# edin-dal/sdqlpy

Hardware: AMD Instinct MI355X
Metric: tpch_q1_q3_q5_sf10_rows_per_sec (higher is better)
Workload: dtype f64; 1 GPU; TPCH Q1+Q3+Q5 SF=10 per GPU (BASELINE metric: Q1/Q3/Q5 at SF=10; q1 = configs[1], q3 = configs[2]); partitioning=none

## Files before the change

sdqlpy_amd/csrc/sdqh_hip.hip:

```cpp
#include <hip/hip_runtime.h>

#include <algorithm>
#include <atomic>
#include <chrono>
#include <cmath>
#include <cstdio>
#include <cstdlib>
#include <cstring>
#include <string>
#include <thread>
#include <type_traits>
#include <map>
#include <vector>

#include "sdqh_host.hpp"

using namespace sdqh_host;

static int ensure_index(sdqh_ctx* ctx, sdqh_table* tb);

namespace sdqh_host {

int fail(sdqh_ctx* ctx, int code, const std::string& msg) {
    if (ctx) ctx->err = msg;
    return code;
}

void* pool_alloc(sdqh_ctx* ctx, size_t bytes) {
    bytes = std::max<size_t>(256, (bytes + 255) & ~(size_t)255);
    int best = -1;
    for (size_t i = 0; i < ctx->pool.size(); ++i) {
        PoolBlock& b = ctx->pool[i];
        if (b.free && b.size >= bytes && b.size <= bytes * 2 + (1u << 20) && (best < 0 || b.size < ctx->pool[(size_t)best].size)) best = (int)i;
    }
    if (best >= 0) { PoolBlock& b = ctx->pool[(size_t)best]; b.free = false; b.alloc_seq = ctx->launch_seq; b.fill_use = false; b.graph_owner = ctx->capturing ? ctx->capture_tag : nullptr; return b.ptr; }
    void* p = nullptr;
    if (hipMalloc(&p, bytes) != hipSuccess) {
        for (auto& b : ctx->pool) if (b.free && b.ptr) { (void)hipFree(b.ptr); b.ptr = nullptr; }
        ctx->pool.erase(std::remove_if(ctx->pool.begin(), ctx->pool.end(), [](const PoolBlock& b) { return b.ptr == nullptr; }), ctx->pool.end());
        if (hipMalloc(&p, bytes) != hipSuccess) { (void)hipGetLastError(); return nullptr; }
    }
    { PoolBlock nb{p, bytes, false}; nb.alloc_seq = ctx->launch_seq; nb.graph_owner = ctx->capturing ? ctx->capture_tag : nullptr; ctx->pool.push_back(nb); }
    return p;
}
void pool_free(sdqh_ctx* ctx, void* p) {
    if (!p) return;
    for (auto& b : ctx->pool) if (b.ptr == p) { if (b.graph_owner) return; b.free = true; for (int h = 0; h < b.nhabits; ++h) b.habits[h].clean = false; if (!b.fill_use) b.nhabits = 0; return; }
}

void* attach_alloc(sdqh_ctx* ctx, const sdqh_column* c, size_t bytes) {
    sdqh_ctx* h = c->home ? c->home : ctx;
    if (h != ctx && h->stream) (void)hipStreamSynchronize(h->stream);
    return pool_alloc(h, bytes);
}
void attach_free(sdqh_ctx* ctx, const sdqh_column* c, void* p) { pool_free(c->home ? c->home : ctx, p); }

hipEvent_t next_event(sdqh_ctx* ctx) {
    if (ctx->event_next == ctx->event_pool.size()) { hipEvent_t e; (void)hipEventCreate(&e); ctx->event_pool.push_back(e); }
    return ctx->event_pool[ctx->event_next++];
}
void call_begin(sdqh_ctx* ctx) {
    if (ctx->nested) return;
    if (ctx->profiling != 2) { ctx->prof.clear(); ctx->event_next = 0; }
    ctx->call_timed = false;
    if (ctx->profiling != 1) return;
    (void)hipEventRecord(ctx->call_begin, ctx->stream);
}
void call_end(sdqh_ctx* ctx) {
    if (ctx->nested || ctx->profiling != 1) return;
    (void)hipEventRecord(ctx->call_end, ctx->stream);
    ctx->call_timed = true;
}

int sync_stream(sdqh_ctx* ctx) {
    if (ctx->capturing) return fail(ctx, SDQH_ERR_UNSUPPORTED, "a call that waits for the device cannot be recorded into a plan graph");
    bool done = false;
    if (ctx->opt_spin_sync && !ctx->compile_only) {
        if (!ctx->sync_flag) {
            void* p = nullptr;
            if (hipHostMalloc(&p, 64, hipHostMallocDefault) == hipSuccess) { ctx->sync_flag = static_cast<volatile uint32_t*>(p); *ctx->sync_flag = 0; }
            else { (void)hipGetLastError(); ctx->opt_spin_sync = 0; }
        }
        if (ctx->sync_flag) {
            const uint32_t seq = ++ctx->sync_seq;
            if (hipStreamWriteValue32(ctx->stream, const_cast<uint32_t*>(ctx->sync_flag), seq, 0) == hipSuccess) {
// ... 515 lines not shown
    if (!ctx || !ms) return SDQH_ERR_INVALID;
    if (!ctx->call_timed) { *ms = 0.0; return SDQH_OK; }
    HIP_TRY(ctx, hipEventSynchronize(ctx->call_end));
    float f = 0;
    HIP_TRY(ctx, hipEventElapsedTime(&f, ctx->call_begin, ctx->call_end));
    *ms = f;
    return SDQH_OK;
}
int sdqh_set_profiling(sdqh_ctx* ctx, int mode) {
    if (!ctx || mode < 0 || mode > 2) return SDQH_ERR_INVALID;
    ctx->profiling = mode; ctx->prof.clear(); ctx->event_next = 0;
    return SDQH_OK;
}
int sdqh_set_profile_filter(sdqh_ctx* ctx, const char* kernel_name) {
    if (!ctx) return SDQH_ERR_INVALID;
    ctx->prof_filter = kernel_name ? kernel_name : "";
    return SDQH_OK;
}
int sdqh_profile_count(const sdqh_ctx* ctx) { return ctx ? (int)ctx->prof.size() : 0; }
int sdqh_profile_entry(const sdqh_ctx* cctx, int i, const char** name, double* ms) {
    sdqh_ctx* ctx = const_cast<sdqh_ctx*>(cctx);
    if (!ctx || i < 0 || i >= (int)ctx->prof.size() || !name || !ms) return SDQH_ERR_INVALID;
    ProfEntry& e = ctx->prof[(size_t)i];
    if (e.ms == 0.0) { (void)hipEventSynchronize(e.e1); float f = 0; if (hipEventElapsedTime(&f, e.e0, e.e1) == hipSuccess) e.ms = f; }
    *name = e.name; *ms = e.ms;
    return SDQH_OK;
}
int sdqh_profile_entry_bytes(const sdqh_ctx* ctx, int i, int64_t* model_bytes) {
    if (!ctx || i < 0 || i >= (int)ctx->prof.size() || !model_bytes) return SDQH_ERR_INVALID;
    *model_bytes = ctx->prof[(size_t)i].model_bytes;
    return SDQH_OK;
}
void* sdqh_stream(const sdqh_ctx* ctx) { if (ctx) const_cast<sdqh_ctx*>(ctx)->stream_exported = true; return ctx ? (void*)ctx->stream : nullptr; }
int sdqh_set_option(sdqh_ctx* ctx, const char* name, int64_t value) {
    if (!ctx || !name) return SDQH_ERR_INVALID;
    const std::string n(name);
    if (n == "resident_cap" && value >= 1 && value <= 8) ctx->opt_resident_cap = (int)value;
    else if (n == "async_copies" && (value == 0 || value == 1)) ctx->opt_async_copies = (int)value;
    else if (n == "resident_stream" && value >= 1 && value <= 8) ctx->opt_resident_stream = (int)value;
    else if (n == "probe_chunk" && value >= 1 && value <= 64) ctx->opt_probe_chunk = (int)value;
    else if (n == "probe_unroll" && (value == 1 || value == 2 || value == 4)) ctx->opt_probe_unroll = (int)value;
    else if (n == "stage_batch" && (value == 2 || value == 4 || value == 8)) ctx->opt_stage_batch = (int)value;
    else if (n == "stage_eager" && (value == 0 || value == 1)) ctx->opt_stage_eager = (int)value;
    else if (n == "stage_eager_pay" && (value == 0 || value == 1)) ctx->opt_stage_eager_pay = (int)value;
    else if (n == "stage_waves_per_cu" && value >= 4 && value <= 64) ctx->opt_stage_waves_per_cu = (int)value;
    else if (n == "direct_index" && (value == 0 || value == 1)) ctx->opt_direct_index = (int)value;
    else if (n == "row_pack" && (value == 0 || value == 1)) ctx->opt_row_pack = (int)value;
    else if (n == "cluster_pack" && value >= 0 && value <= 2) ctx->opt_cluster_pack = (int)value;
    else if (n == "cluster_list" && (value == 0 || value == 1)) ctx->opt_cluster_list = (int)value;
    else if (n == "x_driven" && value >= 0 && value <= (1 << 20)) ctx->opt_x_driven = (int)value;
    else if (n == "delta8" && (value == 0 || value == 1)) ctx->opt_delta8 = (int)value;
    else if (n == "word_pairs" && (value == 0 || value == 1)) ctx->opt_word_pairs = (int)value;
    else if (n == "coarse_kb" && value >= 0 && value <= 96) ctx->opt_coarse_kb = (int)value;
    else if (n == "lookup_pipeline" && value >= -1 && value <= 1) ctx->opt_lookup_pipeline = (int)value;
    else if (n == "probe_pipeline" && value >= 0 && value <= 1) ctx->opt_probe_pipeline = (int)value;
    else if (n == "lookup_debug") ctx->opt_lookup_debug = (int)value;
    else if (n == "fuse_small" && value >= 0 && value <= 1) ctx->opt_fuse_small = (int)value;
    else if (n == "lds_key_set" && value >= 0 && value <= 1) ctx->opt_lds_key_set = (int)value;
    else if (n == "fill_ahead" && value >= 0 && value <= 1) { ctx->opt_fill_ahead = (int)value; for (auto& b : ctx->pool) b.nhabits = 0; }
    else if (n == "str_rows" && (value == 0 || value == 32 || value == 64)) ctx->opt_str_rows = (int)value;
    else if (n == "rank_increasing" && value >= 0 && value <= 1) ctx->opt_rank_increasing = (int)value;
    else if (n == "feature_min_rows" && value >= 0) ctx->opt_feature_min_rows = value;
    else if (n == "narrow" && value >= 0 && value <= 1) ctx->opt_narrow = (int)value;
    else if (n == "tight" && value >= 0 && value <= 1) ctx->opt_tight = (int)value;
    else if (n == "spin_sync" && value >= 0 && value <= 1) ctx->opt_spin_sync = (int)value;
    else if (n == "vstage" && value >= 0 && value <= 1) ctx->opt_vstage = (int)value;
    else if (n == "side_streams" && value >= 0 && value <= 1) ctx->opt_side_streams = (int)value;
    else if (n == "side_priority" && value >= 0 && value <= 1) ctx->opt_side_priority = (int)value;
    else if (n == "copy_kernel" && value >= 0 && value <= 4096) ctx->opt_copy_kernel = (int)value;
    else if (n == "copy_nt" && value >= 0 && value <= 1) ctx->opt_copy_nt = (int)value;
    else if (n == "x_waves" && value >= 0 && value <= 256) ctx->opt_x_waves = (int)value;
    else if (n == "window" && value >= 0 && value <= 1) ctx->opt_window = (int)value;
    else if (n == "lane_int" && value >= 0 && value <= 1) ctx->opt_lane_int = (int)value;
    else if (n == "row_index" && value >= 0 && value <= 1) ctx->opt_row_index = (int)value;
    else if (n == "lane_resident" && value >= 1 && value <= 4) ctx->opt_lane_resident = (int)value;
    else if (n == "async_result" && value >= 0 && value <= 1) ctx->opt_async_result = (int)value;
    else if (n == "stage_pipeline" && value >= 0 && value <= 1) ctx->opt_stage_pipeline = (int)value;
    else if (n == "span_index" && value >= 0 && value <= 1) ctx->opt_span_index = (int)value;
    else if (n == "dense_increasing" && value >= 0 && value <= 1) ctx->opt_dense_increasing = (int)value;
    else if (n == "packed_slots" && (value == 0 || value == 1)) ctx->opt_packed_slots = (int)value;
    else if (n == "grouped_index" && (value == 0 || value == 1)) ctx->opt_grouped_index = (int)value;
    else if (n == "grouped_pairs" && (value == 0 || value == 1)) ctx->opt_grouped_pairs = (int)value;
    else if (n == "index_inline" && (value == 0 || value == 1)) ctx->opt_index_inline = (int)value;
    else if (n == "groupby_regs" && (value == 0 || value == 4 || value == 8)) ctx->opt_groupby_regs = (int)value;
    else if (n == "hash_filter" && (value == 0 || value == 1)) ctx->opt_hash_filter = (int)value;
    else if (n == "pack_ordered" && (value == 0 || value == 1)) ctx->opt_pack_ordered = (int)value;
    else if (n == "pool_trim" && value == 1) {
        if (ctx->compile_only) return SDQH_OK;
        if (ctx->capturing) return fail(ctx, SDQH_ERR_UNSUPPORTED, "set_option: pool_trim inside a recording");
        (void)hipSetDevice(ctx->device);
        if (hipStreamSynchronize(ctx->stream) != hipSuccess) { (void)hipGetLastError(); return fail(ctx, SDQH_ERR_DEVICE, "pool_trim: the stream failed"); }
        for (auto& b : ctx->pool) if (b.free && b.ptr && !b.graph_owner) { (void)hipFree(b.ptr); b.ptr = nullptr; }
        ctx->pool.erase(std::remove_if(ctx->pool.begin(), ctx->pool.end(), [](const PoolBlock& b) { return b.ptr == nullptr; }), ctx->pool.end());
    }
    else return fail(ctx, SDQH_ERR_INVALID, "set_option: unknown option or value out of range: " + n);
    return SDQH_OK;
}

int sdqh_memory_stats(sdqh_ctx* ctx, int64_t* out, int n) {
    if (!ctx || !out || n < 4) return fail(ctx, SDQH_ERR_INVALID, "memory_stats: bad arguments");
    int64_t used = 0, cached = 0, graphs = 0, blocks = 0;
    for (const auto& b : ctx->pool) {
        if (!b.ptr) continue;
        ++blocks;
        if (b.graph_owner) graphs += (int64_t)b.size;
        if (b.free && !b.graph_owner) cached += (int64_t)b.size; else used += (int64_t)b.size;
    }
    out[0] = used; out[1] = cached; out[2] = graphs; out[3] = blocks;
    return SDQH_OK;
}

static int new_column(sdqh_ctx* ctx, int64_t nrows, int dtype, int width, sdqh_column** out) {
    if (!ctx || !out || nrows < 0) return fail(ctx, SDQH_ERR_INVALID, "column: bad arguments");
    if (dtype != SDQH_I64 && dtype != SDQH_F64 && dtype != SDQH_STR) return fail(ctx, SDQH_ERR_INVALID, "column: bad dtype");
    if (dtype == SDQH_STR && width < 1) return fail(ctx, SDQH_ERR_INVALID, "column: STR needs width >= 1");
    sdqh_column* c = new sdqh_column();
    c->home = ctx;
    c->nrows = nrows; c->dtype = dtype; c->width = dtype == SDQH_STR ? width : 0;
    *out = c;
    return SDQH_OK;
}

int sdqh_column_alloc(sdqh_ctx* ctx, int64_t nrows, int dtype, int width, sdqh_column** out) {
    if (int rc = new_column(ctx, nrows, dtype, width, out)) return rc;
    sdqh_column* c = *out;
    (void)hipSetDevice(ctx->device);
    c->data = pool_alloc(ctx, (size_t)nrows * c->row_bytes() + 64);
    c->owned = true;
    if (!c->data) { delete c; *out = nullptr; return fail(ctx, SDQH_ERR_NOMEM, "column_alloc: out of device memory"); }
    return SDQH_OK;
}

static void staging_copy(void* dst, const void* src, size_t n) {
    const unsigned hw = std::thread::hardware_concurrency();
    const size_t parts = n < ((size_t)4 << 20) ? 1 : std::min<size_t>(8, std::max<unsigned>(1, hw / 2));
    if (parts <= 1) { std::memcpy(dst, src, n); return; }
    std::vector<std::thread> th;
    const size_t per = ((n / parts) + 4095) & ~(size_t)4095;
    for (size_t k = 1; k < parts; ++k) {
        const size_t b = std::min(n, k * per), e = std::min(n, (k + 1) * per);
        if (e > b) th.emplace_back([=] { std::memcpy(static_cast<char*>(dst) + b, static_cast<const char*>(src) + b, e - b); });
    }
    std::memcpy(dst, src, std::min(n, per));
    for (auto& t : th) t.join();
}

int sdqh_column_upload(sdqh_ctx* ctx, const void* host, int64_t nrows, int dtype, int width, sdqh_column** out) {
    if (nrows > 0 && !host) return fail(ctx, SDQH_ERR_INVALID, "column_upload: null host pointer");
    if (int rc = sdqh_column_alloc(ctx, nrows, dtype, width, out)) return rc;
    sdqh_column* c = *out;
    const size_t bytes = (size_t)nrows * c->row_bytes();
    size_t off = 0; int i = 0;
    while (off < bytes) {
        const size_t n = std::min(STAGING_BYTES, bytes - off);
        if (ctx->staging_busy[i]) { HIP_TRY(ctx, hipEventSynchronize(ctx->staging_done[i])); ctx->staging_busy[i] = false; }
        staging_copy(ctx->staging[i], static_cast<const char*>(host) + off, n);
        HIP_TRY(ctx, hipMemcpyAsync(static_cast<char*>(c->data) + off, ctx->staging[i], n, hipMemcpyHostToDevice, ctx->stream));
        HIP_TRY(ctx, hipEventRecord(ctx->staging_done[i], ctx->stream));
        ctx->staging_busy[i] = true;
        off += n; i ^= 1;
    }
    for (int k = 0; k < 2; ++k) if (ctx->staging_busy[k]) { HIP_TRY(ctx, hipEventSynchronize(ctx->staging_done[k])); ctx->staging_busy[k] = false; }
    return SDQH_OK;
}

int sdqh_column_wrap(sdqh_ctx* ctx, void* device_ptr, int64_t nrows, int dtype, int width, sdqh_column** out) {
// ... 252 lines not shown
        const int g = order[i];
        if (out_keys) for (int k = 0; k < nkeys; ++k) out_keys[i * nkeys + k] = (int64_t)((hk[g] >> (32 * k)) & 0xFFFFFFFFull);
        if (out_values) for (int k = 0; k < SDQH_TUPLE_MAX_VALUES; ++k) out_values[i * SDQH_TUPLE_MAX_VALUES + k] = k < nv ? ha[g * 4 + k] : 0.0;
        if (out_counts) out_counts[i] = hc[g];
    }
    *out_ngroups = ng;
    return SDQH_OK;
}

static void table_release(sdqh_ctx* ctx, sdqh_table* t) {
    for (void* p : t->owned) pool_free(ctx, p);
    t->owned.clear();
}
static void* table_alloc(sdqh_ctx* ctx, sdqh_table* t, size_t bytes) {
    void* p = pool_alloc(ctx, bytes);
    if (p) t->owned.push_back(p);
    return p;
}

static int setup_stage(sdqh_ctx* ctx, sdqh_table* tb, int64_t nrows, const sdqh_column* key, int npay, const sdqh_column* const* payload, int batch, int waves_per_cu = 24) {
    DevStage& st = tb->stage;
    std::memset(&st, 0, sizeof(st));
    const int64_t target_segs = (int64_t)ctx->num_cu * waves_per_cu;
    int64_t seg_rows = (nrows + target_segs - 1) / target_segs;
    const int64_t gran = (int64_t)WAVE * ROWS_PER_LOAD * std::max(1, batch);
    seg_rows = std::max<int64_t>(gran, (seg_rows + gran - 1) / gran * gran);
    if (seg_rows >= ((int64_t)1 << 31)) return fail(ctx, SDQH_ERR_UNSUPPORTED, "build: more than 2^31 rows per staging segment");
    st.seg_rows = seg_rows;
    st.nseg = (int32_t)std::max<int64_t>(1, (nrows + seg_rows - 1) / seg_rows);
    st.npay = npay;
    const size_t col_bytes = (size_t)std::max<int64_t>(nrows, 1) * 8 + 64;
    st.key = static_cast<int64_t*>(table_alloc(ctx, tb, col_bytes));
    st.src_key = static_cast<const int64_t*>(key->data);
    bool ok = st.key != nullptr;
    for (int p = 0; p < npay && ok; ++p) {
        st.pay[p] = static_cast<int64_t*>(table_alloc(ctx, tb, col_bytes));
        st.src_pay[p] = static_cast<const int64_t*>(payload[p]->data);
        ok = st.pay[p] != nullptr;
    }
    st.seg_count = static_cast<uint32_t*>(table_alloc(ctx, tb, (size_t)st.nseg * 4 + 64));
    st.shits = static_cast<uint32_t*>(table_alloc(ctx, tb, (size_t)std::max<int64_t>(nrows, 1) * 4 + 64));
    ok = ok && st.seg_count != nullptr && st.shits != nullptr;
    st.acc_stride = 4;
    if (ok && tb->accumulate) { st.sacc = static_cast<double*>(table_alloc(ctx, tb, (size_t)std::max<int64_t>(nrows, 1) * 32 + 64)); ok = st.sacc != nullptr; }
    if (!ok) return fail(ctx, SDQH_ERR_NOMEM, "out of device memory for the build stage");
    return SDQH_OK;
}

static void prefill_refs(sdqh_ctx* ctx, sdqh_table* tb, FillList* fl) {
    if (!tb->bm || tb->dev.bm_shift != 0) return;
    const size_t rows = (size_t)std::max<int64_t>(tb->nrows_build, 1);
    if (rows * 4 > ((size_t)8 << 20)) return;
    uint32_t* dense = static_cast<uint32_t*>(table_alloc(ctx, tb, rows * 4 + 64));
    if (!dense) return;
    tb->dev.dense_ref = dense; tb->refs_prefilled = true;
    fl->add(dense, (rows * 4 + 15) & ~(size_t)15, 0xFF);
    const size_t range = (size_t)tb->nwords * 32;
    if (ctx->opt_span_index && tb->dev.lin_rb == 0 && range * 4 <= ((size_t)2 << 20)) {
        uint32_t* span = static_cast<uint32_t*>(table_alloc(ctx, tb, range * 4 + 64));
        if (span) { tb->span = span; fl->add(span, range * 4, 0xFF); }
    }
}

static int ensure_index(sdqh_ctx* ctx, sdqh_table* tb) {
    if (tb->index_built || tb->bitmap_only) return SDQH_OK;
    if (tb->dev.grp_first) { tb->index_built = true; return SDQH_OK; }
    const unsigned seg_grid = (unsigned)((tb->stage.nseg + TPB / WAVE - 1) / (TPB / WAVE));
    const size_t rows = (size_t)std::max<int64_t>(tb->nrows_build, 1);
    if (tb->bm && tb->dev.bm_shift == 0 && tb->stage.wrow) {
        LAUNCH(ctx, "k_wrow_fixup", k_wrow_fixup, (unsigned)((tb->stage.nseg + TPB - 1) / TPB), tb->stage, tb->wexc, tb->hdr);
        tb->dev.wprefix = tb->stage.wrow; tb->dev.dense_ref = nullptr; tb->dev.wexc = tb->wexc;
        hipError_t er = hipGetLastError();
        if (er != hipSuccess) return fail(ctx, SDQH_ERR_DEVICE, std::string("table index launch: ") + hipGetErrorString(er));
        tb->index_built = true;
        return SDQH_OK;
    }
    if (tb->bm && tb->dev.bm_shift == 0) {
        const int nblocks = (int)((tb->nwords + RANK_BLOCK_WORDS - 1) / RANK_BLOCK_WORDS);
        uint32_t* wprefix = static_cast<uint32_t*>(table_alloc(ctx, tb, tb->nwords * 4 + 64));
        uint32_t* dense = tb->refs_prefilled ? tb->dev.dense_ref : static_cast<uint32_t*>(table_alloc(ctx, tb, rows * 4 + 64));
        if (!wprefix || !dense) return fail(ctx, SDQH_ERR_NOMEM, "table index: out of device memory");
        tb->dev.wprefix = wprefix; tb->dev.dense_ref = dense;
        if (nblocks == 1 && seg_grid == 1 && tb->refs_prefilled && ctx->opt_fuse_small) {
            LAUNCH(ctx, "k_index_small", k_index_small, 1u, tb->bm, tb->nwords, wprefix, tb->stage, tb->dev, tb->span);
            if (tb->span) tb->dev.dense_arr = tb->span;
            hipError_t es = hipGetLastError();
            if (es != hipSuccess) return fail(ctx, SDQH_ERR_DEVICE, std::string("table index launch: ") + hipGetErrorString(es));
            tb->index_built = true;
            return SDQH_OK;
        }
        if (nblocks == 1 && ctx->opt_fuse_small && (tb->refs_prefilled || tb->keys_unique) && tb->nwords <= (uint64_t)RANK_BLOCK_WORDS) {
            LAUNCH(ctx, "k_index_medium", k_index_medium, seg_grid, tb->bm, (uint32_t)tb->nwords, wprefix, tb->stage, tb->dev, tb->span);
            if (tb->span) tb->dev.dense_arr = tb->span;
            hipError_t em = hipGetLastError();
            if (em != hipSuccess) return fail(ctx, SDQH_ERR_DEVICE, std::string("table index launch: ") + hipGetErrorString(em));
            tb->index_built = true;
            return SDQH_OK;
        }
        LAUNCH(ctx, "k_rank_words", k_rank_words, (unsigned)nblocks, tb->bm, tb->nwords, wprefix, tb->stage.seg_count, tb->stage.nseg, tb->hdr);
        if (!tb->refs_prefilled && !tb->keys_unique) LAUNCH(ctx, "k_fill_refs", k_fill_refs, (unsigned)ctx->num_cu * 2, tb->stage, tb->dev);
        LAUNCH(ctx, "k_insert_direct", k_insert_direct, seg_grid, tb->stage, tb->dev, tb->span);
        if (tb->span) tb->dev.dense_arr = tb->span;
    } else {
        const bool packed = ctx->opt_packed_slots && tb->npay >= 1 && tb->capmax <= (1ull << 27);
        int64_t* keys = nullptr; uint32_t* rowref = nullptr; int64_t* slots = nullptr;
        if (packed) slots = static_cast<int64_t*>(table_alloc(ctx, tb, (tb->capmax + 2) * 32));
        else { keys = static_cast<int64_t*>(table_alloc(ctx, tb, (tb->capmax + 2) * 8)); rowref = static_cast<uint32_t*>(table_alloc(ctx, tb, (tb->capmax + 2) * 4)); }
        if (packed ? !slots : (!keys || !rowref)) return fail(ctx, SDQH_ERR_NOMEM, "table index: out of device memory");
        tb->dev.keys = keys; tb->dev.rowref = rowref; tb->dev.slots = slots;
        uint32_t* hf = nullptr;
        if (ctx->opt_hash_filter) {
            const uint64_t bits = std::max<uint64_t>(std::min<uint64_t>(tb->capmax, HF_MAX_CAP) << HF_SHIFT, 1024);
            hf = static_cast<uint32_t*>(table_alloc(ctx, tb, (size_t)(bits / 8) + 64));
            if (!hf) (void)hipGetLastError();
        }
        tb->dev.hf = hf;
        LAUNCH(ctx, "k_clear", k_clear, (unsigned)ctx->num_cu * 4, tb->stage.seg_count, tb->stage.nseg, tb->capmax, tb->hdr, keys, rowref, slots, hf);
        LAUNCH(ctx, "k_insert", k_insert, seg_grid, tb->stage, tb->dev);
        LAUNCH(ctx, "k_insert_fixup", k_insert_fixup, seg_grid, tb->stage, tb->dev);
        if (packed) LAUNCH(ctx, "k_insert_repack", k_insert_repack, seg_grid, tb->stage, tb->dev);
    }
    hipError_t e = hipGetLastError();
    if (e != hipSuccess) return fail(ctx, SDQH_ERR_DEVICE, std::string("table index launch: ") + hipGetErrorString(e));
    tb->index_built = true;
    return SDQH_OK;
}

static int build_dense(sdqh_ctx* ctx, int64_t nrows, const sdqh_column* key, int npayload, const sdqh_column* const* payload,
                       int64_t lo, int64_t hi, int accumulate, sdqh_table** out) {
    sdqh_table* tb = new sdqh_table();
    tb->npay = npayload; tb->nrows_build = nrows; tb->index_built = true; tb->accumulate = accumulate != 0;
    DevStage& st = tb->stage;
    std::memset(&st, 0, sizeof(st));
    const int64_t target_segs = (int64_t)ctx->num_cu * ctx->opt_stage_waves_per_cu;
    const int64_t gran = (int64_t)WAVE * ROWS_PER_LOAD * 8;
    int64_t seg_rows = (nrows + target_segs - 1) / target_segs;
    st.seg_rows = std::max<int64_t>(gran, (seg_rows + gran - 1) / gran * gran);
    st.nseg = (int32_t)std::max<int64_t>(1, (nrows + st.seg_rows - 1) / st.seg_rows);
    st.npay = npayload;
    st.key = const_cast<int64_t*>(static_cast<const int64_t*>(key->data));
    for (int p = 0; p < npayload; ++p) st.pay[p] = const_cast<int64_t*>(static_cast<const int64_t*>(payload[p]->data));
    const uint64_t range = (uint64_t)(hi - lo) + 1;
    st.seg_count = static_cast<uint32_t*>(table_alloc(ctx, tb, (size_t)st.nseg * 4 + 64));
    st.shits = static_cast<uint32_t*>(table_alloc(ctx, tb, (size_t)nrows * 4 + 64));
    tb->hdr = static_cast<TableHeader*>(table_alloc(ctx, tb, sizeof(TableHeader)));
    const size_t acc_bytes = accumulate ? (size_t)nrows * 32 : 0;
    if (accumulate) {
        st.acc_stride = 4;
        st.sacc = static_cast<double*>(table_alloc(ctx, tb, acc_bytes + 64));
        if (!st.sacc) { table_release(ctx, tb); delete tb; return fail(ctx, SDQH_ERR_NOMEM, "dense build: out of device memory"); }
        tb->dev.sacc = st.sacc; tb->dev.acc_stride = 4;
    }
    const bool increasing = ctx->opt_dense_increasing && column_is_increasing(ctx, const_cast<sdqh_column*>(key));
    const int64_t* kc = static_cast<const int64_t*>(key->data);
    const unsigned grid = (unsigned)std::min<int64_t>((nrows + TPB - 1) / TPB, (int64_t)ctx->num_cu * 8);
    if (increasing && ctx->opt_rank_increasing && (range * 4 > ((uint64_t)16 << 20) || ctx->opt_feature_min_rows == 0)) {
        tb->nwords = (range + 31) / 32;
        tb->bm = static_cast<uint32_t*>(table_alloc(ctx, tb, tb->nwords * 4 + 64));
        uint32_t* wprefix = static_cast<uint32_t*>(table_alloc(ctx, tb, tb->nwords * 4 + 64));
        uint32_t* wpair = ctx->opt_word_pairs ? static_cast<uint32_t*>(table_alloc(ctx, tb, tb->nwords * 8 + 64)) : nullptr;
        if (!st.seg_count || !st.shits || !tb->hdr || !tb->bm || !wprefix) { table_release(ctx, tb); delete tb; return fail(ctx, SDQH_ERR_NOMEM, "dense build: out of device memory"); }
        st.hdr = tb->hdr;
        tb->dev.hdr = tb->hdr; tb->dev.shits = st.shits; tb->dev.bm_lo = lo; tb->dev.bm_hi = hi; tb->dev.bm = tb->bm; tb->dev.bm_shift = 0; tb->dev.wprefix = wprefix;
        tb->dev.wpair = reinterpret_cast<const unsigned long long*>(wpair);
        for (int p = 0; p < npayload; ++p) tb->dev.pay[p] = st.pay[p];
        call_begin(ctx);
        { FillList fl; fl.add(tb->hdr, sizeof(TableHeader), 0); fl.add(st.shits, (size_t)nrows * 4, 0); fl.add(tb->bm, tb->nwords * 4, 0); if (wpair) fl.add(wpair, tb->nwords * 8, 0); if (accumulate) fl.add(st.sacc, acc_bytes, 0); launch_fill(ctx, fl); }
// ... 752 lines not shown
int sdqh_build(sdqh_ctx* ctx, int64_t nrows, const sdqh_filter* filter, int nlookups, const sdqh_lookup* lookups,
               int nkey, const sdqh_source* key, int npayload, const sdqh_source* payload, int accumulate, sdqh_table** out) {
    if (!ctx || nrows < 0 || !out || nkey < 1 || nkey > 2 || !key || npayload < 0 || npayload > SDQH_MAX_PAYLOAD || (npayload && !payload))
        return fail(ctx, SDQH_ERR_INVALID, "build: bad arguments");
    if (nrows >= 0xFFFFFFFEll) return fail(ctx, SDQH_ERR_UNSUPPORTED, "build: build side limited to 2^32-2 rows per GPU");
    (void)hipSetDevice(ctx->device);
    DevFilter f; DevLookups L; DevBuildSpec spec;
    std::memset(&spec, 0, sizeof(spec));
    bool composite = nkey == 2;
    if (int rc = make_filter(ctx, nrows, filter, nullptr, &f)) return rc;
    call_begin(ctx);
    if (int rc = make_lookups(ctx, nrows, nlookups, lookups, &L, &composite)) return rc;
    spec.nkey = nkey; spec.npay = npayload;
    for (int k = 0; k < nkey; ++k) if (int rc = make_source(ctx, key[k], nrows, nlookups, lookups, nlookups, "build key", &spec.key[k])) return rc;
    for (int p = 0; p < npayload; ++p) if (int rc = make_source(ctx, payload[p], nrows, nlookups, lookups, nlookups, "build payload", &spec.pay[p])) return rc;
    int64_t lo = 0, hi = -1; bool want_bm = false;
    if (nrows > 0 && key[0].kind == SDQH_SRC_COLUMN && key[0].col->dtype == SDQH_I64) {
        if (int rc = ensure_minmax(ctx, const_cast<sdqh_column*>(key[0].col))) return rc;
        lo = key[0].col->mn; hi = key[0].col->mx;
        if (hi >= lo && lo > INT64_MIN / 2 && hi < INT64_MAX / 2) {
            const uint64_t range = (uint64_t)(hi - lo) + 1;
            want_bm = range <= (1ull << 31) && range <= 64ull * (uint64_t)std::max<int64_t>(nrows, 1024);
            if (nkey == 2 && (lo < 0 || hi > 0xFFFFFFFFll)) want_bm = false;
        }
    }
    int64_t lin_rb = 0, lin_b0 = 0; uint64_t lin_bits = 0;
    if (want_bm && nkey == 2 && ctx->opt_direct_index && key[1].kind == SDQH_SRC_COLUMN && key[1].col->dtype == SDQH_I64) {
        if (int rc = ensure_minmax(ctx, const_cast<sdqh_column*>(key[1].col))) return rc;
        const int64_t blo = key[1].col->mn, bhi = key[1].col->mx;
        if (bhi >= blo && blo >= 0 && bhi <= 0xFFFFFFFFll) {
            const uint64_t ra = (uint64_t)(hi - lo) + 1, rb = (uint64_t)(bhi - blo) + 1;
            if (rb <= (1ull << 31) / ra && ra * rb <= 64ull * (uint64_t)std::max<int64_t>(nrows, 1024)) { lin_rb = (int64_t)rb; lin_b0 = blo; lin_bits = ra * rb; }
        }
    }
    const bool grouped = ctx->opt_grouped_index && ctx->opt_direct_index && want_bm && nkey == 2 && !lin_rb && nrows > 1 && nrows < ((int64_t)1 << 31) &&
                         hi < ((int64_t)1 << 31) && !key[0].col->transient && column_is_nondecreasing(ctx, const_cast<sdqh_column*>(key[0].col));
    sdqh_table* tb = new sdqh_table();
    tb->npay = npayload; tb->accumulate = accumulate != 0; tb->nrows_build = nrows;
    if (nkey == 1 && nrows > 0 && key[0].kind == SDQH_SRC_COLUMN && key[0].col->dtype == SDQH_I64 && column_is_increasing(ctx, const_cast<sdqh_column*>(key[0].col))) tb->keys_unique = true;
    if (nkey == 2 && nrows > 0 && key[0].kind == SDQH_SRC_COLUMN && key[1].kind == SDQH_SRC_COLUMN && key[0].col->nrows == nrows && key[1].col->nrows == nrows &&
        columns_pair_increasing(ctx, const_cast<sdqh_column*>(key[0].col), const_cast<sdqh_column*>(key[1].col))) tb->pack_unique = true;
    sdqh_column fake; fake.data = nullptr;
    const sdqh_column* fakes[SDQH_MAX_PAYLOAD] = {&fake, &fake, &fake, &fake};
    int rc = setup_stage(ctx, tb, nrows, &fake, npayload, fakes, nrows >= (int64_t)ctx->num_cu * 24 * 512 ? BUILD_LB : 1);
    uint64_t capmax = 1024;
    while (capmax < 2 * (uint64_t)std::max<int64_t>(nrows, 1)) capmax <<= 1;
    tb->capmax = capmax;
    int* flags = nullptr;
    if (!rc) {
        tb->hdr = static_cast<TableHeader*>(table_alloc(ctx, tb, sizeof(TableHeader)));
        flags = static_cast<int*>(table_alloc(ctx, tb, 64));
        if (want_bm && ctx->opt_direct_index) { tb->nwords = lin_rb ? (lin_bits + 31) / 32 : ((uint64_t)(hi - lo) + 32) / 32; tb->bm = static_cast<uint32_t*>(table_alloc(ctx, tb, tb->nwords * 4 + 64)); }
        if (!tb->hdr || !flags || (tb->nwords && !tb->bm)) rc = fail(ctx, SDQH_ERR_NOMEM, "build: out of device memory");
    }
    uint32_t* grp_first = nullptr;
    const size_t grp_cells = grouped ? (size_t)(hi - lo) + 1 : 0;
    if (!rc && grouped && tb->bm) grp_first = static_cast<uint32_t*>(table_alloc(ctx, tb, grp_cells * 4 + 64));
    if (!rc) {
        tb->dev.hdr = tb->hdr; tb->dev.shits = tb->stage.shits; tb->dev.sacc = tb->stage.sacc; tb->dev.acc_stride = tb->stage.acc_stride;
        if (grp_first) {
            tb->stage.grp_first = grp_first;
            tb->dev.grp_first = grp_first; tb->dev.grp_key = tb->stage.key; tb->dev.grp_kstride = 1; tb->dev.grp_seg_rows = tb->stage.seg_rows;
            if (npayload >= 1 && ctx->opt_grouped_pairs) {
                int64_t* kp = static_cast<int64_t*>(table_alloc(ctx, tb, ((size_t)nrows + 8) * 16 + 64));
                if (kp) { tb->stage.grp_kp = kp; tb->dev.grp_key = kp; tb->dev.grp_kstride = 2; }
            } tb->dev.grp_cap = nrows + 1;
        }
        const int shift = (nkey == 2 && !(tb->bm && lin_rb)) ? 32 : 0;
        tb->dev.bm = tb->bm; tb->dev.bm_lo = lo; tb->dev.bm_hi = hi; tb->dev.bitmap_only = 0; tb->dev.bm_shift = shift;
        for (int p = 0; p < npayload; ++p) tb->dev.pay[p] = tb->stage.pay[p];
        tb->stage.bm = tb->bm; tb->stage.bm_lo = lo; tb->stage.bm_hi = hi; tb->stage.hdr = tb->hdr; tb->stage.bm_shift = shift;
        if (tb->bm && lin_rb) { tb->dev.lin_rb = tb->stage.lin_rb = lin_rb; tb->dev.lin_b0 = tb->stage.lin_b0 = lin_b0; }
        const unsigned seg_grid = (unsigned)((tb->stage.nseg + TPB / WAVE - 1) / (TPB / WAVE));
        FillList fl; fl.add(tb->hdr, sizeof(TableHeader), 0); fl.add(flags, 8, 0); if (tb->bm) fl.add(tb->bm, tb->nwords * 4, 0); prefill_refs(ctx, tb, &fl);
        if (grp_first) fl.add(grp_first, grp_cells * 4, 0xFF);
        DevFill pre; std::memset(&pre, 0, sizeof(pre));
        prune_clean(ctx, &fl);
        if (seg_grid == 1 && ctx->opt_fuse_small && fl.most <= ((uint64_t)1 << 20) && fl.f.n <= FILL_MAX) pre = fl.pre(); else launch_fill(ctx, fl);
        DevIndexInline ix; std::memset(&ix, 0, sizeof(ix));
        if (seg_grid == 1 && ctx->opt_fuse_small && ctx->opt_index_inline && tb->bm && shift == 0 && tb->refs_prefilled && (tb->nwords + RANK_BLOCK_WORDS - 1) / RANK_BLOCK_WORDS == 1) {
            uint32_t* wprefix = static_cast<uint32_t*>(table_alloc(ctx, tb, tb->nwords * 4 + 64));
            if (wprefix) {
                tb->dev.wprefix = wprefix;
                ix.t = tb->dev; ix.wprefix = wprefix; ix.span = tb->span; ix.nwords = tb->nwords; ix.on = 1;
            }
        }
        hipError_t e;
        with_scan_filter(f, [&](auto FC) {
            using FCT = decltype(FC);
            if constexpr (std::is_same_v<FCT, FCfg<1, 0, 0, 0>> || std::is_same_v<FCT, FCfg<0, 0, 0, 0>>) {
                const bool eager0 = nlookups > 0 && lookups[0].key[0].kind == SDQH_SRC_COLUMN && lookups[0].key[0].col->dtype == SDQH_I64;
                if (ctx->opt_narrow && nrows >= ctx->opt_feature_min_rows && (eager0 || f.ni == 1)) {
                    const int32_t* nkey0 = eager0 ? static_cast<const int32_t*>(ensure_narrow(ctx, const_cast<sdqh_column*>(lookups[0].key[0].col))) : nullptr;
                    const int32_t* npred0 = f.ni == 1 ? static_cast<const int32_t*>(ensure_narrow(ctx, const_cast<sdqh_column*>(filter->ipred[0].col))) : nullptr;
                    if ((!eager0 || nkey0) && (f.ni != 1 || npred0)) {
                        auto kern = k_build_lookup<FCT, true>;
                        LAUNCH(ctx, "k_build_lookup", kern, seg_grid, f, L, spec, tb->stage, nrows, flags, nkey0, npred0, pre, ix);
                        return SDQH_OK;
                    }
                }
            }
            auto kern = k_build_lookup<FCT>;
            LAUNCH(ctx, "k_build_lookup", kern, seg_grid, f, L, spec, tb->stage, nrows, flags, static_cast<const int32_t*>(nullptr), static_cast<const int32_t*>(nullptr), pre, ix);
            return SDQH_OK;
        });
        if (ix.on) { if (tb->span) tb->dev.dense_arr = tb->span; tb->index_built = true; }
        call_end(ctx);
        e = hipGetLastError();
        if (e != hipSuccess) rc = fail(ctx, SDQH_ERR_DEVICE, std::string("build launch: ") + hipGetErrorString(e));
        auto packs = [&](const sdqh_source& src) {
            if (src.kind != SDQH_SRC_COLUMN || !src.col || src.col->dtype != SDQH_I64) return false;
            sdqh_column* c = const_cast<sdqh_column*>(src.col);
            return ensure_minmax(ctx, c) == SDQH_OK && c->nrows > 0 && c->mn >= 0 && c->mx <= 0xFFFFFFFFll;
        };
        bool proven = composite;
        if (composite && !rc) {
            if (nkey == 2) proven = proven && packs(key[0]) && packs(key[1]);
            for (int l = 0; l < nlookups && proven; ++l) if (lookups[l].nkey == 2) proven = packs(lookups[l].key[0]) && packs(lookups[l].key[1]);
        }
        if (!rc && composite && !proven) {
            e = hipMemcpyAsync(ctx->result_host, flags, 4, hipMemcpyDeviceToHost, ctx->stream);
            if (e != hipSuccess) rc = fail(ctx, SDQH_ERR_DEVICE, hipGetErrorString(e));
            if (!rc) rc = sync_stream(ctx);
            if (!rc && (*static_cast<const int*>(ctx->result_host) & 2)) rc = fail(ctx, SDQH_ERR_UNSUPPORTED, "build: composite key part outside [0, 2^32)");
        }
    }
    if (rc) { table_release(ctx, tb); delete tb; return rc; }
    *out = tb;
    return SDQH_OK;
}

static int lookup_aggregate_launch(sdqh_ctx* ctx, int64_t nrows, const sdqh_filter* filter, int nlookups, const sdqh_lookup* lookups,
                                   int nkeys, const sdqh_source* keys, int tuple_shape, const sdqh_source* operands, void* block, bool device_block) {
    (void)hipSetDevice(ctx->device);
    const int nops = tuple_nops(tuple_shape), nv = tuple_nv(tuple_shape);
    if (nops < 0) return fail(ctx, SDQH_ERR_UNSUPPORTED, "unknown tuple shape");
    DevFilter f; DevLookups L; DevAggSpec spec;
    std::memset(&spec, 0, sizeof(spec));
    bool composite = false;
    if (int rc = make_filter(ctx, nrows, filter, nullptr, &f)) return rc;
    call_begin(ctx);
    if (int rc = make_lookups(ctx, nrows, nlookups, lookups, &L, &composite)) return rc;
    spec.nkeys = nkeys; spec.shape = tuple_shape;
    for (int k = 0; k < nkeys; ++k) if (int rc = make_source(ctx, keys[k], nrows, nlookups, lookups, nlookups, "group key", &spec.key[k])) return rc;
    for (int j = 0; j < nops; ++j) if (int rc = make_source(ctx, operands[j], nrows, nlookups, lookups, nlookups, "tuple operand", &spec.op[j])) return rc;
    L.debug = ctx->opt_lookup_debug;
    L.pipeline = 0;
    if (nlookups > 0 && lookups[0].key[0].kind == SDQH_SRC_COLUMN && lookups[0].key[0].col->dtype == SDQH_I64)
        L.pipeline = ctx->opt_lookup_pipeline >= 0 ? ctx->opt_lookup_pipeline : (column_is_clustered(ctx, const_cast<sdqh_column*>(lookups[0].key[0].col)) ? 1 : 0);
    const int32_t* cluster_key32 = nullptr;
    size_t coarse_lds = 0;
    if (ctx->opt_row_pack && nlookups > 0 && nrows > 0 && nrows >= ctx->opt_feature_min_rows) {
        std::vector<DevSource*> srcs;
        for (int l = 0; l < nlookups; ++l) for (int k = 0; k < L.l[l].nkey; ++k) srcs.push_back(&L.l[l].key[k]);
        for (int k = 0; k < nkeys; ++k) srcs.push_back(&spec.key[k]);
        for (int j = 0; j < nops; ++j) srcs.push_back(&spec.op[j]);
        std::vector<const void*> cols;
        for (DevSource* sr : srcs) if (sr->kind == SDQH_SRC_COLUMN && std::find(cols.begin(), cols.end(), (const void*)sr->col) == cols.end()) cols.push_back(sr->col);
        if (cols.size() >= 5 && cols.size() <= (size_t)MAX_PACK && (size_t)nrows * cols.size() * 8 <= ((size_t)48 << 30)) {
            const int k = (int)((cols.size() + 1) & ~(size_t)1);
            const void* order_col = nullptr;
            sdqh_column* kc0 = (lookups[0].key[0].kind == SDQH_SRC_COLUMN && lookups[0].key[0].col->dtype == SDQH_I64) ? const_cast<sdqh_column*>(lookups[0].key[0].col) : nullptr;
            const sdqh_table* t0 = lookups[0].table;
            const bool unfiltered = f.nc == 0 && f.ns == 0 && f.nf == 0 && f.ni == 0;
            const bool part_bm = t0->bm && !t0->dev.lin_rb && (lookups[0].nkey == 1 ? t0->dev.bm_shift == 0 : t0->dev.bm_shift != 0);
            if (ctx->opt_cluster_pack && ctx->opt_narrow && kc0 && unfiltered && part_bm && !kc0->transient && nrows < ((int64_t)1 << 32) &&
                (nrows >= 4 * ctx->opt_feature_min_rows || ctx->opt_feature_min_rows == 0) && (ctx->opt_cluster_pack == 2 || !column_is_clustered(ctx, kc0)) && ensure_minmax(ctx, kc0) == SDQH_OK)
                order_col = kc0->data;
            sdqh_ctx::RowPack* found = nullptr;
// ... 523 lines not shown
```

sdqlpy_amd/csrc/sdqh_host.hpp:

```cpp
#pragma once
#include <hip/hip_runtime.h>

#include <atomic>
#include <map>
#include <string>
#include <vector>

#include "sdqh.h"
#include "sdqh_kernels.hpp"

namespace sdqh_host {

struct FillHabit { size_t off, bytes; int byte; bool clean; };
struct PoolBlock {
    void* ptr; size_t size; bool free;
    FillHabit habits[4] = {};
    int nhabits = 0;
    uint64_t alloc_seq = 0;
    bool fill_use = false;
    const void* graph_owner = nullptr;
};
struct ProfEntry { const char* name; hipEvent_t e0, e1; double ms; int64_t model_bytes; };

constexpr size_t STAGING_BYTES = 32u << 20;
constexpr size_t RESULT_BYTES = 64u << 10;

}

using namespace sdqh;

struct sdqh_ctx {
    int device = 0;
    sdqh_ctx* parent = nullptr;
    std::vector<sdqh_ctx*> children;
    const void* capture_tag = nullptr;
    struct HostInit { void* p; uint64_t value; int bytes; };
    std::vector<HostInit> capture_inits;
    bool capturing = false;
    bool dying = false;
    bool compile_only = false;
    int num_cu = 256;
    hipStream_t stream = nullptr;
    bool stream_exported = false;
    std::string err;
    std::vector<sdqh_host::PoolBlock> pool;
    void* staging[2] = {nullptr, nullptr};
    hipEvent_t staging_done[2] = {nullptr, nullptr};
    bool staging_busy[2] = {false, false};
    void* result_host = nullptr;
    void* result_dev = nullptr;
    void* bulk_host = nullptr;
    size_t bulk_bytes = 0;
    std::map<const char*, size_t> host_blocks;
    void* count_host = nullptr;
    hipEvent_t call_begin = nullptr, call_end = nullptr;
    bool call_timed = false;
    int profiling = 0;
    std::string prof_filter;
    std::vector<sdqh_host::ProfEntry> prof;
    int64_t next_model_bytes = 0;
    std::vector<hipEvent_t> event_pool;
    size_t event_next = 0;
    const void* lds_hint[SDQH_MAX_GROUPKEYS] = {nullptr, nullptr};
    int threads = 1;
    std::vector<std::pair<const void*, int>> occupancy;
    int opt_resident_cap = 6;
    int opt_async_copies = 0;
    int opt_probe_chunk = 1;
    int opt_resident_stream = 2;
    int opt_probe_unroll = PROBE_UNROLL;
    int opt_stage_batch = STAGE_BATCH;
    int opt_stage_eager = 1;
    int nested = 0;
    int opt_stage_eager_pay = 0;
    int opt_stage_waves_per_cu = 12;
    int opt_direct_index = 1;
    int opt_packed_slots = 1;
    int opt_lookup_pipeline = -1;
    int opt_lookup_debug = 0;
    size_t rd_clean_ff = 0; int64_t rd_clean_zero_off = -1;
    int opt_fill_ahead = 1;
    uint64_t launch_seq = 0;
    int opt_lds_key_set = 1;
    int opt_fuse_small = 1;
    int opt_str_rows = 0;
    int opt_rank_increasing = 1;
    int64_t opt_feature_min_rows = 1 << 20;
    bool in_groupby_key = false;
    int opt_vstage = 1;
    int opt_tight = 1;
    hipStream_t side[2] = {nullptr, nullptr};
    hipEvent_t side_ev[4] = {nullptr, nullptr, nullptr, nullptr};
    int opt_side_streams = 1;
    int opt_side_priority = 1;
    int opt_copy_kernel = 0;
    int opt_copy_nt = 1;
    int opt_row_index = 1;
    int opt_grouped_index = 1;
    int opt_grouped_pairs = 1;
    int opt_index_inline = 1;
    int opt_lane_int = 1;
    int opt_lane_resident = 2;
    int opt_window = 0;
    int opt_x_driven = 64;
    int opt_word_pairs = 0;
    int opt_delta8 = 1;
    int opt_x_waves = 0;
    void* rs_dev[2] = {nullptr, nullptr}; size_t rs_bytes[2] = {0, 0};
    hipEvent_t rs_copied[2] = {nullptr, nullptr}; bool rs_used[2] = {false, false};
    int rs_cur = 0; bool rs_pending = false;
    hipEvent_t rs_ready = nullptr;
    volatile uint32_t* sync_flag = nullptr; uint32_t sync_seq = 0; int opt_spin_sync = 1;
    int opt_async_result = 1;
    int opt_narrow = 1;
    int opt_stage_pipeline = 0;
    int opt_span_index = 1;
    int opt_dense_increasing = 1;
    int opt_probe_pipeline = 0;
    const void* coarse_stat_col = nullptr; uint64_t* coarse_stat = nullptr;
    unsigned long long* coarse_count_dev = nullptr; uint64_t coarse_stat_bits_pending = 0; int coarse_skipped = 0; int64_t coarse_stat_build_rows = -1;
    int opt_coarse_kb = 64;
    int opt_row_pack = 1;
    struct RowPack { std::vector<const void*> cols; int64_t nrows; int k; void* data; const void* order_col = nullptr; void* key32 = nullptr;
                     void* lb = nullptr; int64_t key_lo = 0, key_hi = -1; };
    std::vector<RowPack> packs;
    int opt_pack_ordered = 1;
    int opt_hash_filter = 1;
    int opt_cluster_list = 1;
    int opt_cluster_pack = 1;
    int opt_groupby_regs = 0;
    const void* g4_hint[SDQH_MAX_GROUPKEYS] = {nullptr, nullptr};
};

inline uint64_t sdqh_next_uid() { static std::atomic<uint64_t> next{1}; return next.fetch_add(1, std::memory_order_relaxed); }

struct sdqh_column {
    uint64_t uid = sdqh_next_uid();
    uint64_t pair_uid = 0; int pair_increasing = -1;
    sdqh_ctx* home = nullptr;
    void* data = nullptr;
    int64_t nrows = 0;
    int dtype = SDQH_I64;
    int width = 0;
    bool owned = false;
    long long* d_minmax = nullptr;
    bool minmax_pending = false, have_minmax = false;
    int clustered = -1;
    void* narrow = nullptr;
    int narrow_state = -1;
    int increasing = -1;
    int nondecreasing = -1;
    int span8 = -1;
    int64_t mn = 0, mx = 0;
    void* code = nullptr;
    int code_width = 0;
    int code_state = -1;
    void* dict = nullptr;
    int ndict = 0;
    std::vector<int64_t> dict_host;
    void* delta8 = nullptr;
    int delta8_state = -1;
    void* run_index = nullptr;
    int run_index_state = -1;
    bool transient = false;
    size_t row_bytes() const { return dtype == SDQH_STR ? (size_t)width * 4 : 8; }
};

struct sdqh_table {
    sdqh::DevTable dev{};
    DevStage stage{};
    TableHeader* hdr = nullptr;
    uint32_t* bm = nullptr;
    int npay = 0;
    bool accumulate = false;
    bool bitmap_only = false;
    int64_t nrows_build = 0;
    uint64_t capmax = 0;
    bool index_built = false;
    uint64_t nwords = 0;
    std::vector<void*> owned;
    uint32_t* span = nullptr;
    bool pack_unique = false;
    bool keys_unique = false;
// ... 86 lines not shown
```

sdqlpy_amd/csrc/sdqh_kernels.hpp:

```cpp
#pragma once
#ifndef __HIPCC_RTC__
#include <hip/hip_runtime.h>
#include <stdint.h>
#endif
#include "sdqh.h"

#if defined(__HIPCC_RTC__) || defined(SDQH_DECLS_ONLY)
#define SDQH_KERNEL template <int SDQH_RTC_UNUSED = 0> __global__
#else
#define SDQH_KERNEL __global__
#endif

namespace sdqh {

constexpr int TPB = 256;
constexpr int WAVE = 64;
constexpr int ROWS_PER_LOAD = 2;
#ifndef SDQH_UNROLL
#define SDQH_UNROLL 2
#endif
#ifndef SDQH_NT_LOADS
#define SDQH_NT_LOADS 1
#endif
#ifndef SDQH_TILE_CHUNK
// ... 1206 lines not shown
                const int off = j * (int)BATCH_ROWS + lane * ROWS_PER_LOAD;
                if (p[j][0]) q_off[at] = (uint16_t)off;
                if (p[j][1]) q_off[at + (p[j][0] ? 1 : 0)] = (uint16_t)(off + 1);
                qn += __popcll(b0) + __popcll(b1);
            }
            __builtin_amdgcn_wave_barrier();
            for (int i0 = 0; i0 < qn; i0 += WAVE) {
                const int i = i0 + lane;
                if (i < qn) {
                    const int64_t row = b + q_off[i];
                    int64_t pay[MAX_STAGE_COLS];
                    const int64_t key = st.src_key[row];
#pragma unroll
                    for (int c = 0; c < MAX_STAGE_COLS; ++c) pay[c] = c < cfg_npay<NPAY>(st.npay) ? st.src_pay[c][row] : 0;
                    stage_store<NPAY>(st, out + i, key, pay);
                }
            }
            __builtin_amdgcn_wave_barrier();
            out += qn;
            continue;
        }
        if (!(EAGER_PAY && full_step)) {
#pragma unroll
            for (int j = 0; j < SB; ++j) {
#pragma unroll
                for (int q = 0; q < 2; ++q) {
                    kx[j][q] = p[j][q] ? st.src_key[r[j] + q] : 0;
#pragma unroll
                    for (int c = 0; c < MAX_STAGE_COLS; ++c) px[j][q][c] = (c < cfg_npay<NPAY>(st.npay) && p[j][q]) ? st.src_pay[c][r[j] + q] : 0;
                }
            }
        }
#pragma unroll
        for (int j = 0; j < SB; ++j) {
            const uint64_t b0 = __ballot(p[j][0]), b1 = __ballot(p[j][1]);
            const int64_t pos0 = out + __popcll(b0 & lt) + __popcll(b1 & lt);
            if (p[j][0]) stage_store<NPAY>(st, pos0, kx[j][0], px[j][0]);
            if (p[j][1]) stage_store<NPAY>(st, pos0 + (p[j][0] ? 1 : 0), kx[j][1], px[j][1]);
            out += __popcll(b0) + __popcll(b1);
        }
    }
    if (lane == 0) st.seg_count[seg] = (uint32_t)(out - begin);
}

SDQH_KERNEL __launch_bounds__(TPB) void k_clear(const uint32_t* __restrict__ seg_count, int nseg, uint64_t capmax,
                                               TableHeader* __restrict__ hdr, int64_t* __restrict__ keys, uint32_t* __restrict__ rowref, int64_t* __restrict__ slots,
                                               uint32_t* __restrict__ hf) {
    __shared__ unsigned long long s_part[TPB];
    unsigned long long t = 0;
    for (int i = threadIdx.x; i < nseg; i += TPB) t += seg_count[i];
    s_part[threadIdx.x] = t;
    __syncthreads();
    for (int off = TPB / 2; off > 0; off >>= 1) { if ((int)threadIdx.x < off) s_part[threadIdx.x] += s_part[threadIdx.x + off]; __syncthreads(); }
    const uint64_t staged = s_part[0];
    uint64_t cap = 1024;
    while (cap < 2 * staged) cap <<= 1;
    if (cap > capmax) cap = capmax;
    if (blockIdx.x == 0 && threadIdx.x == 0) {
        hdr->cap_mask = cap - 1; hdr->staged = staged;
        if (slots) { slots[cap * 4] = EMPTY_KEY; slots[cap * 4 + 3] = (int64_t)NO_ROW; }
        else { keys[cap] = EMPTY_KEY; rowref[cap] = NO_ROW; }
    }
    if (hf) {
        using W = uint32_t __attribute__((ext_vector_type(4)));
        const uint32_t hm = hf_mask_of(cap - 1);
        const uint64_t n16 = ((uint64_t)hm + 1) / 128;
        const uint32_t z = hm == HF_DEGENERATE ? 0xFFFFFFFFu : 0u;
        const W zero = {z, z, z, z};
        W* h4 = reinterpret_cast<W*>(hf);
        for (uint64_t i = (uint64_t)blockIdx.x * TPB + threadIdx.x; i < n16; i += (uint64_t)gridDim.x * TPB) h4[i] = zero;
    }
    using V = long long __attribute__((ext_vector_type(2)));
    if (slots) {
        const V a = {(long long)EMPTY_KEY, 0}, b = {0, (long long)NO_ROW};
        V* s2 = reinterpret_cast<V*>(slots);
        for (uint64_t i = (uint64_t)blockIdx.x * TPB + threadIdx.x; i < cap; i += (uint64_t)gridDim.x * TPB) { s2[2 * i] = a; s2[2 * i + 1] = b; }
        return;
    }
    const V empty = {(long long)EMPTY_KEY, (long long)EMPTY_KEY};
    V* k2 = reinterpret_cast<V*>(keys);
    for (uint64_t i = (uint64_t)blockIdx.x * TPB + threadIdx.x; i < cap / 2; i += (uint64_t)gridDim.x * TPB) k2[i] = empty;
}

__device__ __forceinline__ void rank_words_body(const uint32_t* __restrict__ bm, uint64_t nwords, uint32_t* __restrict__ wprefix,
                                                const uint32_t* __restrict__ seg_count, int nseg, TableHeader* __restrict__ hdr) {
    __shared__ uint32_t s_wave[TPB / WAVE];
    __shared__ uint32_t s_base;
    constexpr int ROWS = RANK_BLOCK_WORDS / (TPB * 4);
    const uint64_t q0 = (uint64_t)blockIdx.x * (RANK_BLOCK_WORDS / 4);
    const uint64_t nquads = (nwords + 3) / 4;
    const int w = threadIdx.x / WAVE, lane = lane_id();
    uint4 quad[ROWS];
    uint32_t excl[ROWS];
    uint32_t running = 0;
#pragma unroll
    for (int r = 0; r < ROWS; ++r) {
        const uint64_t qi = q0 + (uint64_t)r * TPB + threadIdx.x;
        uint4 a = make_uint4(0u, 0u, 0u, 0u);
        if (qi < nquads) {
            a = *reinterpret_cast<const uint4*>(bm + qi * 4);
            const uint64_t wi = qi * 4;
            if (wi + 1 >= nwords) a.y = 0u;
            if (wi + 2 >= nwords) a.z = 0u;
            if (wi + 3 >= nwords) a.w = 0u;
        }
        quad[r] = a;
        const uint32_t mine = (uint32_t)(__popc(a.x) + __popc(a.y) + __popc(a.z) + __popc(a.w));
        uint32_t incl = mine;
#pragma unroll
        for (int off = 1; off < WAVE; off <<= 1) { const uint32_t v = __shfl_up(incl, off, WAVE); if (lane >= off) incl += v; }
        __syncthreads();
        if (lane == WAVE - 1) s_wave[w] = incl;
        __syncthreads();
        uint32_t before = 0, total = 0;
#pragma unroll
        for (int i = 0; i < TPB / WAVE; ++i) { if (i < w) before += s_wave[i]; total += s_wave[i]; }
        excl[r] = running + before + incl - mine;
        running += total;
    }
    uint32_t stg = 0;
    for (int i = blockIdx.x * TPB + threadIdx.x; i < nseg; i += gridDim.x * TPB) stg += seg_count[i];
#pragma unroll
    for (int off = WAVE / 2; off > 0; off >>= 1) stg += __shfl_down(stg, off, WAVE);
    if (lane == 0 && stg) atomicAdd(reinterpret_cast<unsigned long long*>(&hdr->staged), (unsigned long long)stg);
    if (threadIdx.x == 0) s_base = running ? (uint32_t)atomicAdd(reinterpret_cast<unsigned long long*>(&hdr->distinct), (unsigned long long)running) : 0u;
    __syncthreads();
    const uint32_t base = s_base;
#pragma unroll
    for (int r = 0; r < ROWS; ++r) {
        const uint64_t qi = q0 + (uint64_t)r * TPB + threadIdx.x;
        if (qi >= nquads) continue;
        uint4 p;
        p.x = base + excl[r];
        p.y = p.x + (uint32_t)__popc(quad[r].x);
        p.z = p.y + (uint32_t)__popc(quad[r].y);
        p.w = p.z + (uint32_t)__popc(quad[r].z);
        *reinterpret_cast<uint4*>(wprefix + qi * 4) = p;
    }
}
SDQH_KERNEL __launch_bounds__(TPB) void k_rank_words(const uint32_t* __restrict__ bm, uint64_t nwords, uint32_t* __restrict__ wprefix,
                                                    const uint32_t* __restrict__ seg_count, int nseg, TableHeader* __restrict__ hdr) {
    rank_words_body(bm, nwords, wprefix, seg_count, nseg, hdr);
}
SDQH_KERNEL __launch_bounds__(TPB) void k_wrow_fixup(DevStage st, WordExc* __restrict__ exc, TableHeader* __restrict__ hdr) {
    const int s = (int)(blockIdx.x * TPB + threadIdx.x);
    if (s == 0) hdr->has_dups = 0;
    if (s >= st.nseg) return;
    const uint32_t cnt = st.seg_count[s];
    if (!cnt) return;
    const SegFirst f = st.seg_first[s];
    const uint64_t off0 = (uint64_t)(f.key - st.bm_lo);
    const uint32_t w0 = (uint32_t)(off0 >> 5), word = st.bm[w0];
    const uint32_t n_below = __popc(word & ((1u << (off0 & 31)) - 1u));
    if (n_below == 0) {
        if (cnt >= (uint32_t)__popc(word)) st.wrow[w0] = f.pos;
        return;
    }
    int t = s - 1;
    while (t > 0 && st.seg_count[t] == 0) --t;
    WordExc e;
    e.key0 = f.key; e.pos0 = f.pos; e.n0 = n_below; e._pad = 0;
    e.pos_prev = (uint32_t)((int64_t)t * st.seg_rows + (int64_t)st.seg_count[t] - (int64_t)n_below);
    exc[s] = e;
    st.wrow[w0] = ROW_INDEX_EXC | (uint32_t)s;
}
__device__ __forceinline__ bool direct_has_dups(const TableHeader* hdr) { return hdr->staged != hdr->distinct; }
SDQH_KERNEL __launch_bounds__(TPB) void k_fill_refs(DevStage st, DevTable t) {
    if (!direct_has_dups(t.hdr)) return;
    const uint64_t n = t.hdr->distinct;
    for (uint64_t i = (uint64_t)blockIdx.x * TPB + threadIdx.x; i < n; i += (uint64_t)gridDim.x * TPB) t.dense_ref[i] = NO_ROW;
}
__device__ __forceinline__ void insert_direct_body(const DevStage& st, const DevTable& t, uint32_t* __restrict__ span) {
    const int seg = blockIdx.x * (TPB / WAVE) + threadIdx.x / WAVE;
    const bool dups = direct_has_dups(t.hdr);
    if (blockIdx.x == 0 && threadIdx.x == 0) t.hdr->has_dups = dups ? 1u : 0u;
    if (seg >= st.nseg) return;
    const int64_t base = (int64_t)seg * st.seg_rows;
    const uint32_t count = st.seg_count[seg];
    for (uint32_t i = lane_id(); i < count; i += WAVE) {
        const int64_t idx = base + i;
        const int64_t pos = table_find(t, st.key[idx], 0);
        if (pos < 0) continue;
        if (dups) atomicMin(&t.dense_ref[pos], (uint32_t)idx); else t.dense_ref[pos] = (uint32_t)idx;
        if (span) { uint32_t* cell = span + (st.key[idx] - t.bm_lo); if (dups) atomicMin(cell, (uint32_t)idx); else *cell = (uint32_t)idx; }
    }
}
SDQH_KERNEL __launch_bounds__(TPB) void k_insert_direct(DevStage st, DevTable t, uint32_t* __restrict__ span) { insert_direct_body(st, t, span); }
SDQH_KERNEL __launch_bounds__(TPB) void k_index_small(const uint32_t* __restrict__ bm, uint64_t nwords, uint32_t* __restrict__ wprefix, DevStage st, DevTable t, uint32_t* __restrict__ span) {
    rank_words_body(bm, nwords, wprefix, st.seg_count, st.nseg, t.hdr);
    __threadfence();
    __syncthreads();
    insert_direct_body(st, t, span);
}
SDQH_KERNEL __launch_bounds__(TPB) void k_index_medium(const uint32_t* __restrict__ bm, uint32_t nwords, uint32_t* __restrict__ wprefix, DevStage st, DevTable t, uint32_t* __restrict__ span) {
    __shared__ uint32_t s_word[RANK_BLOCK_WORDS], s_pre[RANK_BLOCK_WORDS];
    __shared__ uint32_t s_wave[TPB / WAVE];
    __shared__ uint32_t s_staged;
    constexpr int PER = RANK_BLOCK_WORDS / TPB;
    const int lane = lane_id(), w = threadIdx.x / WAVE;
    for (int i = threadIdx.x; i < RANK_BLOCK_WORDS; i += TPB) s_word[i] = (uint32_t)i < nwords ? bm[i] : 0u;
    if (threadIdx.x == 0) s_staged = 0u;
    __syncthreads();
    uint32_t mine = 0;
#pragma unroll
    for (int j = 0; j < PER; ++j) mine += (uint32_t)__popc(s_word[threadIdx.x * PER + j]);
    uint32_t incl = mine;
#pragma unroll
    for (int off = 1; off < WAVE; off <<= 1) { const uint32_t v = __shfl_up(incl, off, WAVE); if (lane >= off) incl += v; }
    if (lane == WAVE - 1) s_wave[w] = incl;
    uint32_t stg = 0;
    for (int i = threadIdx.x; i < st.nseg; i += TPB) stg += st.seg_count[i];
#pragma unroll
    for (int off = WAVE / 2; off > 0; off >>= 1) stg += __shfl_down(stg, off, WAVE);
    if (lane == 0 && stg) atomicAdd(&s_staged, stg);
    __syncthreads();
    uint32_t before = 0, total = 0;
#pragma unroll
    for (int i = 0; i < TPB / WAVE; ++i) { if (i < w) before += s_wave[i]; total += s_wave[i]; }
    uint32_t run = before + incl - mine;
#pragma unroll
    for (int j = 0; j < PER; ++j) { s_pre[threadIdx.x * PER + j] = run; run += (uint32_t)__popc(s_word[threadIdx.x * PER + j]); }
    __syncthreads();
    const uint32_t staged = s_staged;
    const bool dups = staged != total;
    if (blockIdx.x == 0) {
        for (uint32_t i = threadIdx.x; i < nwords; i += TPB) wprefix[i] = s_pre[i];
        if (threadIdx.x == 0) { t.hdr->staged = staged; t.hdr->distinct = total; t.hdr->has_dups = dups ? 1u : 0u; }
    }
    const int seg = blockIdx.x * (TPB / WAVE) + w;
    if (seg >= st.nseg) return;
    const int64_t base = (int64_t)seg * st.seg_rows;
    const uint32_t count = st.seg_count[seg];
    for (uint32_t i = lane; i < count; i += WAVE) {
        const int64_t idx = base + i;
        const int64_t key = st.key[idx];
        uint64_t off;
        if (!bm_locate(t, key, off) || (off >> 5) >= (uint64_t)RANK_BLOCK_WORDS) continue;
        const uint32_t word = s_word[off >> 5];
        if (!((word >> (off & 31)) & 1u)) continue;
        const uint32_t pos = s_pre[off >> 5] + (uint32_t)__popc(word & ((1u << (off & 31)) - 1u));
        if (dups) atomicMin(&t.dense_ref[pos], (uint32_t)idx); else t.dense_ref[pos] = (uint32_t)idx;
        if (span) { uint32_t* cell = span + (key - t.bm_lo); if (dups) atomicMin(cell, (uint32_t)idx); else *cell = (uint32_t)idx; }
    }
}

SDQH_KERNEL __launch_bounds__(TPB) void k_full_counts(uint32_t* __restrict__ seg_count, int nseg, int64_t seg_rows, int64_t nrows) {
    const int s = blockIdx.x * TPB + threadIdx.x;
    if (s < nseg) { int64_t b = (int64_t)s * seg_rows, e = b + seg_rows; if (e > nrows) e = nrows; seg_count[s] = (uint32_t)(e - b); }
}
SDQH_KERNEL __launch_bounds__(TPB) void k_dense_fill(const int64_t* __restrict__ key, int64_t nrows, int64_t lo, uint32_t* __restrict__ arr) {
    for (int64_t r = (int64_t)blockIdx.x * TPB + threadIdx.x; r < nrows; r += (int64_t)gridDim.x * TPB) arr[key[r] - lo] = (uint32_t)r;
}
SDQH_KERNEL __launch_bounds__(TPB) void k_check_increasing(const int64_t* __restrict__ key, int64_t nrows, int* __restrict__ flag) {
    bool bad = false;
    for (int64_t r = (int64_t)blockIdx.x * TPB + threadIdx.x; r + 1 < nrows; r += (int64_t)gridDim.x * TPB) bad |= key[r] >= key[r + 1];
    if (__ballot(bad) && lane_id() == 0) atomicOr(flag, 1);
}
SDQH_KERNEL __launch_bounds__(TPB) void k_check_nondecreasing(const int64_t* __restrict__ key, int64_t nrows, int* __restrict__ flag) {
    bool bad = false;
    for (int64_t r = (int64_t)blockIdx.x * TPB + threadIdx.x; r + 1 < nrows; r += (int64_t)gridDim.x * TPB) bad |= key[r] > key[r + 1];
    if (__ballot(bad) && lane_id() == 0) atomicOr(flag, 1);
}
SDQH_KERNEL __launch_bounds__(TPB) void k_check_pair_increasing(const int64_t* __restrict__ a, const int64_t* __restrict__ b, int64_t nrows, int* __restrict__ flag) {
    bool bad = false;
    for (int64_t r = (int64_t)blockIdx.x * TPB + threadIdx.x; r + 1 < nrows; r += (int64_t)gridDim.x * TPB) bad |= !(a[r] < a[r + 1] || (a[r] == a[r + 1] && b[r] < b[r + 1]));
    if (__ballot(bad) && lane_id() == 0) atomicOr(flag, 1);
}
constexpr int PAIR_RUN_MAX = 32;
SDQH_KERNEL __launch_bounds__(TPB) void k_check_pair_distinct(const int64_t* __restrict__ a, const int64_t* __restrict__ b, int64_t nrows, int* __restrict__ flag) {
    int bad = 0;
    for (int64_t r = (int64_t)blockIdx.x * TPB + threadIdx.x; r + 1 < nrows; r += (int64_t)gridDim.x * TPB) {
        const int64_t ar = a[r], br = b[r];
        int64_t j = r + 1;
        for (; j < nrows && j <= r + PAIR_RUN_MAX && a[j] == ar; ++j) bad |= b[j] == br ? 1 : 0;
        if (j < nrows && j > r + PAIR_RUN_MAX && a[j] == ar) bad |= 2;
// ... 656 lines not shown
    return 0;
}
template <bool PACKED = false>
__device__ __forceinline__ int run_lookups(const DevLookups& L, int64_t r, uint32_t (&ent)[SDQH_MAX_LOOKUP], const PackRow& pr, bool skip0 = false) {
#pragma unroll
    for (int l = 0; l < SDQH_MAX_LOOKUP; ++l) {
        if (l < L.n && !(l == 0 && skip0)) {
            const DevLookup& lk = L.l[l];
            const int64_t p0 = source_value<PACKED>(lk.key[0], L, r, ent, pr);
            const int64_t p1 = lk.nkey == 2 ? source_value<PACKED>(lk.key[1], L, r, ent, pr) : 0;
            int64_t key;
            if (pack_parts(lk.nkey, p0, p1, key)) return -1;
            const uint64_t mask = (table_is_direct(lk.table) || lk.table.bitmap_only) ? 0 : lk.table.hdr->cap_mask;
            const int64_t pos = table_find(lk.table, key, mask);
            if (pos < 0) return 0;
            ent[l] = lk.table.bitmap_only ? 0u : (lk.table.slots && !table_is_direct(lk.table) ? (uint32_t)pos : table_ref(lk.table, pos));
        }
    }
    return 1;
}
__device__ __forceinline__ bool coarse_may_hit(const DevLookups& L, const uint32_t* s_coarse, int64_t part0) {
    const DevTable& t = L.l[0].table;
    if (part0 < t.bm_lo || part0 > t.bm_hi) return false;
    const uint64_t j = (uint64_t)(part0 - t.bm_lo) >> L.coarse_shift;
    return (s_coarse[j >> 5] >> (j & 31)) & 1u;
}
SDQH_KERNEL __launch_bounds__(TPB) void k_coarsen(const uint32_t* __restrict__ bm, uint64_t nbits, int shift, uint32_t* __restrict__ coarse, int cwords, unsigned long long* __restrict__ set_bits) {
    unsigned long long mine = 0;
    for (int w = blockIdx.x * TPB + threadIdx.x; w < cwords; w += gridDim.x * TPB) {
        uint32_t out = 0;
        for (int b = 0; b < 32; ++b) {
            const uint64_t f0 = ((uint64_t)w * 32 + (uint64_t)b) << shift, f1 = f0 + (1ull << shift);
            bool any = false;
            for (uint64_t f = f0; f < f1 && f < nbits && !any; ) {
                const uint32_t word = bm[f >> 5];
                const uint32_t lo = (uint32_t)(f & 31), span = (uint32_t)min((uint64_t)(32 - lo), f1 - f);
                const uint32_t mask = (span >= 32 ? 0xFFFFFFFFu : ((1u << span) - 1u)) << lo;
                any = (word & mask) != 0u;
                f += span;
            }
            out |= any ? (1u << b) : 0u;
        }
        coarse[w] = out;
        mine += (unsigned long long)__popc(out);
    }
    mine = (unsigned long long)wave_sum_i64((long long)mine);
    if (set_bits && lane_id() == 0 && mine) atomicAdd(set_bits, mine);
}
__device__ __forceinline__ bool first_lookup_may_hit(const DevLookups& L, int64_t part0) {
    const DevTable& t = L.l[0].table;
    if (!t.bm) return true;
    if (L.l[0].nkey == 2 && t.bm_shift == 0) return true;
    if (part0 < t.bm_lo || part0 > t.bm_hi) return false;
    const uint64_t off = (uint64_t)(part0 - t.bm_lo);
    return (t.bm[off >> 5] >> (off & 31)) & 1u;
}

__device__ __forceinline__ bool first_lookup_none(const DevLookups& L) {
    const DevTable& t = L.l[0].table;
    return !t.bm || (L.l[0].nkey == 2 && t.bm_shift == 0);
}
__device__ __forceinline__ uint32_t first_lookup_word(const DevLookups& L, int64_t part0) {
    const DevTable& t = L.l[0].table;
    const bool in = part0 >= t.bm_lo && part0 <= t.bm_hi;
    const uint64_t off = in ? (uint64_t)(part0 - t.bm_lo) : 0;
    return t.bm[off >> 5];
}
__device__ __forceinline__ bool first_lookup_bit(const DevLookups& L, int64_t part0, uint32_t word) {
    const DevTable& t = L.l[0].table;
    const bool in = part0 >= t.bm_lo && part0 <= t.bm_hi;
    return in && ((word >> ((uint64_t)(part0 - t.bm_lo) & 31)) & 1u);
}

constexpr int BUILD_LB = 4;
constexpr int LOOKUP_PU = 2;
constexpr int LBQ_CAP = 64 + BUILD_LB * 128;

struct DevBuildSpec {
    int32_t nkey, npay;
    DevSource key[2];
    DevSource pay[SDQH_MAX_PAYLOAD];
};

struct DevIndexInline { DevTable t; uint32_t* wprefix; uint32_t* span; uint64_t nwords; int32_t on, _pad; };

template <class FC, bool NW>
__device__ __forceinline__ void build_lookup_segment(const DevFilter& f, const DevLookups& L, const DevBuildSpec& spec, const DevStage& st, int64_t nrows, int* __restrict__ flags,
                                                     const int32_t* __restrict__ nkey0, const int32_t* __restrict__ npred0, int32_t* q_row, const int seg) {
    const int64_t* skey0 = NW ? reinterpret_cast<const int64_t*>(nkey0) : L.l[0].key[0].col;
    const int64_t begin = (int64_t)seg * st.seg_rows;
    int64_t end = begin + st.seg_rows; if (end > nrows) end = nrows;
    const int lane = lane_id();
    const uint64_t lt = lanemask_lt();
    constexpr int64_t BATCH_ROWS = WAVE * ROWS_PER_LOAD;
    const bool eager0 = L.n > 0 && L.l[0].key[0].kind == SDQH_SRC_COLUMN;
    DevProbes none; none.n = 0;
    const uint64_t nomask[SDQH_MAX_PROBE] = {0, 0};
    int64_t out = begin;
    int qn = 0;
    bool bad = false;
    auto drain = [&](int first, int count) {
        bool keep = false; int64_t key = 0; int64_t pay[MAX_STAGE_COLS] = {0, 0, 0, 0, 0};
        if (lane < count) {
            const int64_t r = begin + (int64_t)q_row[first + lane];
            uint32_t ent[SDQH_MAX_LOOKUP] = {0, 0, 0};
            const PackRow nopack{};
            const int h = run_lookups(L, r, ent, nopack);
            if (h < 0) bad = true;
            if (h > 0) {
                const int64_t p0 = source_value(spec.key[0], L, r, ent, nopack);
                const int64_t p1 = spec.nkey == 2 ? source_value(spec.key[1], L, r, ent, nopack) : 0;
                if (pack_parts(spec.nkey, p0, p1, key)) bad = true;
                else {
                    keep = true;
#pragma unroll
                    for (int q = 0; q < SDQH_MAX_PAYLOAD; ++q) if (q < spec.npay) pay[q] = source_value(spec.pay[q], L, r, ent, nopack);
                }
            }
        }
        const uint64_t b = __ballot(keep);
        bool opens_run = true;
        if (st.grp_first) {
            const uint64_t lower = b & lt;
            const int prev = lower ? 63 - __builtin_clzll(lower) : lane;
            const int64_t prev_key = __shfl(key, prev, WAVE);
            opens_run = !lower || ((uint64_t)prev_key >> 32) != ((uint64_t)key >> 32);
        }
        if (keep) stage_store<-1>(st, out + __popcll(b & lt), key, pay, opens_run);
        out += __popcll(b);
    };
    auto enqueue = [&](int64_t r, bool p0, bool p1) {
        const uint64_t b0 = __ballot(p0), b1 = __ballot(p1);
        if (b0 | b1) {
            const int at = qn + __popcll(b0 & lt) + __popcll(b1 & lt);
            const int32_t off = (int32_t)(r - begin);
            if (p0) q_row[at] = off;
            if (p1) q_row[at + (p0 ? 1 : 0)] = off + 1;
            qn += __popcll(b0) + __popcll(b1);
        }
    };
    for (int64_t b = begin;;) {
        const bool last = b >= end;
        if (last) {
        } else if (b + BATCH_ROWS * BUILD_LB <= end) {
            int64_t rr[BUILD_LB];
            bool p[BUILD_LB][2];
            Pair<int64_t> k0[BUILD_LB];
#pragma unroll
            for (int j = 0; j < BUILD_LB; ++j) {
                rr[j] = b + (int64_t)j * BATCH_ROWS + (int64_t)lane * ROWS_PER_LOAD;
                p[j][0] = p[j][1] = true;
                if (eager0) k0[j] = loadc<false, NW>(skey0, rr[j], nrows);
            }
            pass_pairs<BUILD_LB, FC, false, false, false, NW>(f, none, rr, nrows, nomask, p, nullptr, nullptr, nullptr, npred0);
            if (eager0) {
#pragma unroll
                for (int j = 0; j < BUILD_LB; ++j) { p[j][0] = p[j][0] && first_lookup_may_hit(L, k0[j].x); p[j][1] = p[j][1] && first_lookup_may_hit(L, k0[j].y); }
            }
#pragma unroll
            for (int j = 0; j < BUILD_LB; ++j) enqueue(rr[j], p[j][0], p[j][1]);
            b += BATCH_ROWS * BUILD_LB;
        } else {
            const int64_t r = b + (int64_t)lane * ROWS_PER_LOAD;
            bool p1b[1][2];
            if (b + BATCH_ROWS <= end) {
                int64_t r1[1] = {r};
                p1b[0][0] = p1b[0][1] = true;
                Pair<int64_t> k1 = {0, 0};
                if (eager0) k1 = load2<false>(L.l[0].key[0].col, r, nrows);
                pass_pairs<1, FC, false>(f, none, r1, nrows, nomask, p1b);
                if (eager0) { p1b[0][0] = p1b[0][0] && first_lookup_may_hit(L, k1.x); p1b[0][1] = p1b[0][1] && first_lookup_may_hit(L, k1.y); }
            } else {
                p1b[0][0] = r < end; p1b[0][1] = r + 1 < end;
                if (p1b[0][0]) p1b[0][0] = row_passes<FC>(f, none, r, nomask);
                if (p1b[0][1]) p1b[0][1] = row_passes<FC>(f, none, r + 1, nomask);
            }
            enqueue(r, p1b[0][0], p1b[0][1]);
            b += BATCH_ROWS;
        }
        int head = 0;
        while (qn - head >= WAVE || (last && qn > head)) {
            const int n = qn - head >= WAVE ? WAVE : qn - head;
            drain(head, n);
            head += n;
        }
        if (last) break;
        if (head) {
            const int left = qn - head;
            int32_t keepv = 0;
            if (lane < left) keepv = q_row[head + lane];
            if (lane < left) q_row[lane] = keepv;
            qn = left;
        }
    }
    if (lane == 0) {
        st.seg_count[seg] = (uint32_t)(out - begin);
        stage_end_segment(st, seg, begin, out - begin);
        if (st.grp_first && seg == 0) st.hdr->has_dups = 1u;
    }
    if (__ballot(bad) && lane == 0) atomicOr(flags, 2);
}

template <class FC, bool NW = false>
__global__ __launch_bounds__(TPB) void k_build_lookup(DevFilter f, DevLookups L, DevBuildSpec spec, DevStage st, int64_t nrows, int* __restrict__ flags,
                                                      const int32_t* __restrict__ nkey0, const int32_t* __restrict__ npred0, DevFill pre, DevIndexInline ix) {
    if (pre.n) { fill_in_block(pre); __syncthreads(); }
    __shared__ int32_t s_row[TPB / WAVE][LBQ_CAP];
    const int seg = blockIdx.x * (TPB / WAVE) + threadIdx.x / WAVE;
    if (seg < st.nseg) build_lookup_segment<FC, NW>(f, L, spec, st, nrows, flags, nkey0, npred0, s_row[threadIdx.x / WAVE], seg);
    if (ix.on) {
        __threadfence();
        __syncthreads();
        rank_words_body(st.bm, ix.nwords, ix.wprefix, st.seg_count, st.nseg, st.hdr);
        __threadfence();
        __syncthreads();
        insert_direct_body(st, ix.t, ix.span);
    }
}

struct DevPackCols { const int64_t* col[MAX_PACK]; int32_t ncols, k; };
SDQH_KERNEL __launch_bounds__(TPB) void k_interleave(DevPackCols c, int64_t nrows, int64_t* __restrict__ out) {
    for (int64_t r = (int64_t)blockIdx.x * TPB + threadIdx.x; r < nrows; r += (int64_t)gridDim.x * TPB) {
        int64_t v[MAX_PACK];
#pragma unroll
        for (int j = 0; j < MAX_PACK; ++j) v[j] = j < c.ncols ? c.col[j][r] : 0;
#pragma unroll
        for (int j = 0; j < MAX_PACK; ++j) if (j < c.k) out[r * c.k + j] = v[j];
    }
}

constexpr int LG_SLOTS = 2 * SDQH_MAX_LOOKUP_GROUPS;

struct DevAggSpec {
    int32_t nkeys, shape;
    DevSource key[SDQH_MAX_GROUPKEYS];
    DevSource op[4];
};

__device__ __forceinline__ int group_slot(unsigned long long* keys, unsigned long long key, bool global) {
    int h = (int)(mix64(key) & (LG_SLOTS - 1));
#pragma unroll 1
    for (int i = 0; i < LG_SLOTS; ++i) {
        unsigned long long cur = global ? __hip_atomic_load(&keys[h], __ATOMIC_RELAXED, __HIP_MEMORY_SCOPE_AGENT) : keys[h];
        if (cur == EMPTY_GROUP) cur = atomicCAS(&keys[h], (unsigned long long)EMPTY_GROUP, key);
        if (cur == EMPTY_GROUP || cur == key) return h;
        h = (h + 1) & (LG_SLOTS - 1);
    }
    return -1;
}

template <int SHAPE, class FC, int BT = TPB, int PUV = LOOKUP_PU, bool NW = false, bool WALK = false>
__global__ __launch_bounds__(BT) void k_lookup_agg(DevFilter f, DevLookups L, DevAggSpec spec, int64_t nrows,
                                                    unsigned long long* __restrict__ gkeys, double* __restrict__ pacc,
                                                    int64_t* __restrict__ pcnt, int* __restrict__ flags, int chunk, const int32_t* __restrict__ nkey0) {
    const int64_t* skey0 = NW ? reinterpret_cast<const int64_t*>(nkey0) : L.l[0].key[0].col;
    constexpr int NOPS = TupleTraits<SHAPE>::NOPS, NV = TupleTraits<SHAPE>::NV;
    constexpr int PU = PUV, TILE = BT * ROWS_PER_LOAD * PU, SUBR = BT * ROWS_PER_LOAD, QCAP = 64 + PU * 128;
    __shared__ unsigned long long s_keys[LG_SLOTS];
    constexpr int NVS = NV > 0 ? NV : 1;
    __shared__ double s_acc[LG_SLOTS][NVS];
    __shared__ unsigned long long s_cnt[LG_SLOTS];
    __shared__ int32_t s_row[BT / WAVE][QCAP];
    __shared__ int s_map[LG_SLOTS];
    __shared__ int s_flags[1];
    for (int i = threadIdx.x; i < LG_SLOTS; i += BT) { s_keys[i] = EMPTY_GROUP; s_cnt[i] = 0; for (int k = 0; k < NVS; ++k) s_acc[i][k] = 0.0; s_map[i] = -1; }
    for (int i = threadIdx.x; i < LG_SLOTS; i += BT) pcnt[(size_t)i * gridDim.x + blockIdx.x] = 0;
    if (threadIdx.x == 0) s_flags[0] = 0;
    __syncthreads();
    constexpr bool COARSE = BT != TPB;
    extern __shared__ __align__(16) uint32_t s_coarse[];
    if constexpr (COARSE) { for (int i = threadIdx.x; i < L.coarse_words; i += BT) s_coarse[i] = L.coarse[i]; __syncthreads(); }
    int32_t* q_row = s_row[threadIdx.x / WAVE];
    const int lane = lane_id();
    const uint64_t lt = lanemask_lt();
    const bool eager0 = L.n > 0 && L.l[0].key[0].kind == SDQH_SRC_COLUMN;
    DevProbes none; none.n = 0;
    const uint64_t nomask[SDQH_MAX_PROBE] = {0, 0};
    int qn = 0;
    const bool skip0 = eager0 && !first_lookup_none(L) && L.l[0].table.bitmap_only && L.l[0].nkey == 1 && L.l[0].table.bm_shift == 0 && L.l[0].table.lin_rb == 0 && !(L.debug & 2);
    int64_t qbase = 0;
    auto drain = [&](int first, int count) {
        if (lane >= count) return;
        if (L.debug & 1) return;
        const int64_t r = qbase + (int64_t)q_row[first + lane];
        uint32_t ent[SDQH_MAX_LOOKUP] = {0, 0, 0};
        PackRow prow{};
        if (L.pack) pack_load(L, r, prow);
        double x[4] = {0, 0, 0, 0}, o[4] = {0, 0, 0, 0};
        if (L.debug & 8) { if (prow.v0 == -12345 && prow.v5 == -777) atomicOr(&s_flags[0], 2); return; }
        const int h = run_lookups<true>(L, r, ent, prow, skip0);
        if (h < 0) atomicOr(&s_flags[0], 2);
        if (h <= 0) return;
        if (L.debug & 4) { if (ent[0] + ent[1] + ent[2] == 0xFFFFFFF0u) atomicOr(&s_flags[0], 2); return; }
        const int64_t k0 = source_value<true>(spec.key[0], L, r, ent, prow);
        const int64_t k1 = spec.nkeys == 2 ? source_value<true>(spec.key[1], L, r, ent, prow) : 0;
#pragma unroll
        for (int j = 0; j < NOPS; ++j) x[j] = __longlong_as_double(source_value<true>(spec.op[j], L, r, ent, prow));
        if (k0 < 0 || k0 > 0xFFFFFFFEll || k1 < 0 || k1 > 0xFFFFFFFEll) { atomicOr(&s_flags[0], 2); return; }
        if (!operand_ranges<NOPS>(f, x)) return;
// ... 719 lines not shown
```

sdqlpy_amd/csrc/sdqh_x.hip:

```cpp
#define SDQH_DECLS_ONLY 1
#include <hip/hip_runtime.h>
#include <hip/hiprtc.h>

#include <dlfcn.h>
#include <sys/stat.h>
#include <unistd.h>

#include <algorithm>
#include <chrono>
#include <cstdio>
#include <cstdlib>
#include <cstring>
#include <fstream>
#include <mutex>
#include <sstream>
#include <string>
#include <vector>

#include "sdqh_host.hpp"
#include "sdqh_xkernels.hpp"

using namespace sdqh_host;

namespace {
// ... 1083 lines not shown
    out << "    template <int H> __device__ __forceinline__ static bool eval_regs(const XArgs& a, const Pair<int64_t> (&s)[" << nsx << "], int64_t r, XOut<NV>& o) {\n";
    if (direct) out << body(1, 0); else out << "        return false;\n";
    out << "    }\n";
    out << "    __device__ __forceinline__ static bool eval_row(const XArgs& a, int64_t r, const int64_t (&sres)[" << nsopx << "], XOut<NV>& o) {\n";
    if (!direct) out << body(0, first_gate); else out << "        return false;\n";
    out << "    }\n};\n";
    const std::string sn = sink_name(sink);
    out << "extern \"C\" __global__ __launch_bounds__(256) void " << entry_name(sink, direct, q8) << "(XArgs a, " << sn << "<P::NV>::Args s, int64_t nrows, int64_t seg_rows, int nseg) {\n";
    if (direct) out << "    x_direct<P, " << sn << ">(a, s, nrows);\n";
    else out << "    " << (q8 ? "x_queue8" : "x_queue") << "<P, " << sn << ", " << (sink == SINK_STAGE ? "true" : "false") << ">(a, s, nrows, seg_rows, nseg);\n";
    out << "}\n";
    return out.str();
}

struct JitState {
    std::mutex mu;
    bool headers_loaded = false; std::string h_abi, h_kernels, h_xkernels, src_dir, cache_dir, why_unusable;
    std::map<std::string, hipFunction_t> kernels;
    int64_t compiled = 0, from_disk = 0;
};
JitState& jit() { static JitState s; return s; }

std::string slurp(const std::string& path) {
    std::ifstream f(path, std::ios::binary);
    if (!f) return std::string();
    std::stringstream ss; ss << f.rdbuf();
    return ss.str();
}
uint64_t fnv1a(const std::string& s, uint64_t h = 1469598103934665603ull) {
    for (unsigned char c : s) { h ^= c; h *= 1099511628211ull; }
    return h;
}

bool load_headers(JitState& J) {
    if (J.headers_loaded) return J.why_unusable.empty();
    J.headers_loaded = true;
    std::string dir;
    if (const char* env = std::getenv("SDQLPY_AMD_CSRC")) dir = env;
    else {
        Dl_info info;
        if (dladdr(reinterpret_cast<const void*>(&sdqh_jit_stats), &info) && info.dli_fname) { dir = info.dli_fname; const size_t at = dir.rfind('/'); dir = at == std::string::npos ? "." : dir.substr(0, at); }
    }
    J.src_dir = dir;
    J.h_kernels = slurp(dir + "/sdqh_kernels.hpp");
    J.h_xkernels = slurp(dir + "/sdqh_xkernels.hpp");
    J.h_abi = slurp(dir + "/../../include/sdqh.h");
    if (J.h_abi.empty()) J.h_abi = slurp(dir + "/sdqh.h");
    if (J.h_kernels.empty() || J.h_xkernels.empty() || J.h_abi.empty()) {
        J.why_unusable = "run-time specialisation needs sdqh_kernels.hpp, sdqh_xkernels.hpp next to libsdqlhip.so and include/sdqh.h (looked in " + dir + ")";
        return false;
    }
    if (const char* env = std::getenv("SDQLPY_AMD_JIT_CACHE")) J.cache_dir = env;
    else J.cache_dir = dir + "/../jit_cache";
    (void)mkdir(J.cache_dir.c_str(), 0777);
    return true;
}

uint64_t structure_hash(const XInfo& x, Sink sink, bool direct) {
    const sdqh_program* p = x.p;
    uint64_t h = 1469598103934665603ull;
    auto mix = [&](uint64_t v) { h ^= v; h *= 0x9E3779B97F4A7C15ull; h ^= h >> 29; };
    mix((uint64_t)sink * 2 + (direct ? 1 : 0)); mix((uint64_t)x.narrow_mask);
    if (x.tight) {
        mix(0x7167ull); mix((uint64_t)x.gather32); mix((x.pref32 ? 1ull : 0ull) | (x.vstage ? 2ull : 0ull) | (x.pwin ? 4ull : 0ull) | (x.pnear ? 8ull : 0ull) | (x.driven ? 16ull : 0ull) | (x.phash ? 32ull : 0ull) | ((uint64_t)(x.ival + 1) << 8));
        for (int c = 0; c < x.ncols; ++c) mix(((uint64_t)(uint32_t)x.enc[c] << 32) | ((uint32_t)(x.affine[c] ? 1 : 0) << 16) | (uint32_t)(x.dict_slot[c] & 0xFFFF));
        for (int k = 0; k < x.p->nops; ++k) mix((uint64_t)(uint8_t)x.irange[k]);
        for (int k = 0; k < x.p->nops; ++k) mix(((uint64_t)(uint32_t)x.cmp_cc[k] << 32) | ((uint32_t)x.cmp_kind[k] << 8) | (uint32_t)(x.cmp_col[k] & 0xFF));
    } mix((uint64_t)p->nops); mix((uint64_t)(int64_t)p->key); mix((uint64_t)(int64_t)x.probe_op);
    for (int k = 0; k < p->nops; ++k) {
        const sdqh_xop& o = p->ops[k];
        mix(((uint64_t)(uint32_t)o.code << 32) | (uint32_t)o.type); mix(((uint64_t)(uint32_t)o.a << 32) | (uint32_t)o.b); mix(((uint64_t)(uint32_t)o.c << 32) | (uint32_t)o.aux);
        mix(((uint64_t)(uint32_t)x.col_of[k] << 32) | (uint32_t)x.tab_of[k]); mix(((uint64_t)(uint32_t)x.const_of[k] << 32) | (uint32_t)x.str_off[k]);
        if (o.code == SDQH_X_DIVI || o.code == SDQH_X_MODI) mix((uint64_t)o.imm_i);
        if (o.code == SDQH_X_STR || o.code == SDQH_X_STRIDX) { mix((uint64_t)o.slen); for (int i = 0; i < o.slen; ++i) mix(o.str[i]); }
        if (o.code == SDQH_X_STR || o.code == SDQH_X_STRIDX || o.code == SDQH_X_CHAR) mix((uint64_t)(o.col ? o.col->width : 0));
    }
    mix((uint64_t)p->ngates); for (int g = 0; g < p->ngates; ++g) mix((uint64_t)p->gates[g]);
    mix((uint64_t)p->nvals); for (int v = 0; v < p->nvals; ++v) mix((uint64_t)p->vals[v]);
    return h;
}

int specialise(sdqh_ctx* ctx, const std::string& source, const std::string& entry, hipFunction_t* fn);

int kernel_for(sdqh_ctx* ctx, const XInfo& x, Sink sink, bool direct, hipFunction_t* fn) {
    JitState& J = jit();
    static const bool no_layouts = std::getenv("SDQLPY_AMD_X_NOLAYOUT") != nullptr;
    uint64_t lay_hash = 0;
    for (int t = 0; t < x.ntabs; ++t) {
        if (ctx->compile_only) { x.lay[t] = 0u; continue; }
        if (int rc = index_ensure(ctx, x.tabs[t])) return rc;
        x.lay[t] = no_layouts ? 0u : x_layout_of(x.tabs[t]->dev, x.tabs[t]->bitmap_only);
        lay_hash = (lay_hash ^ x.lay[t]) * 0x9E3779B97F4A7C15ull + (uint64_t)t;
    }
    char name[64];
    std::snprintf(name, sizeof(name), "s%016llx@%d", (unsigned long long)(structure_hash(x, sink, direct) ^ lay_hash), ctx->device);
    if (!ctx->compile_only) {
        std::lock_guard<std::mutex> lock(J.mu);
        auto hit = J.kernels.find(name);
        if (hit != J.kernels.end()) { *fn = hit->second; return SDQH_OK; }
    }
    if (int rc = specialise(ctx, generate(x, sink, direct), (x.vstage && sink == SINK_STAGE) ? std::string(VSTAGE_ENTRY) : entry_name(sink, direct, x.tight), fn)) return rc;
    std::lock_guard<std::mutex> lock(J.mu);
    J.kernels[name] = *fn;
    return SDQH_OK;
}

int specialise(sdqh_ctx* ctx, const std::string& source_in, const std::string& entry, hipFunction_t* fn) {
    std::string source = source_in;
    if (const char* defs = std::getenv("SDQLPY_AMD_X_DEFINES")) {
        std::istringstream in(defs); std::string tok, head;
        while (in >> tok) { const size_t eq = tok.find('='); head += "#define " + (eq == std::string::npos ? tok + " 1" : tok.substr(0, eq) + " " + tok.substr(eq + 1)) + "\n"; }
        source = head + source;
    }
    JitState& J = jit();
    std::lock_guard<std::mutex> lock(J.mu);
    if (!load_headers(J)) return fail(ctx, SDQH_ERR_DEVICE, J.why_unusable);
    int rtc_major = 0, rtc_minor = 0;
    (void)hiprtcVersion(&rtc_major, &rtc_minor);
    uint64_t h = fnv1a(source);
    h = fnv1a(J.h_xkernels, h); h = fnv1a(J.h_kernels, h); h = fnv1a(J.h_abi, h);
    h = fnv1a("gfx950 rtc " + std::to_string(rtc_major) + "." + std::to_string(rtc_minor), h);
    char name[64];
    std::snprintf(name, sizeof(name), "%016llx", (unsigned long long)h);
    const std::string key = std::string(name) + "@" + std::to_string(ctx->device);
    auto hit = J.kernels.find(key);
    if (hit != J.kernels.end()) { *fn = hit->second; return SDQH_OK; }
    if (const char* dump = std::getenv("SDQLPY_AMD_JIT_DUMP")) if (dump[0] == '2') std::fprintf(stderr, "---- specialised source (%s) ----\n%s\n", entry.c_str(), source.c_str());
    const std::string path = J.cache_dir + "/" + name + ".hsaco";
    std::string code = slurp(path);
    if (!code.empty()) ++J.from_disk;
    else {
        hiprtcProgram prog;
        const char* hs[3] = {J.h_abi.c_str(), J.h_kernels.c_str(), J.h_xkernels.c_str()};
        const char* hn[3] = {"sdqh.h", "sdqh_kernels.hpp", "sdqh_xkernels.hpp"};
        if (hiprtcCreateProgram(&prog, source.c_str(), "sdqh_specialised.hip", 3, hs, hn) != HIPRTC_SUCCESS)
            return fail(ctx, SDQH_ERR_DEVICE, "hiprtcCreateProgram failed");
        const char* opts[] = {"--offload-arch=gfx950", "-O3", "-std=c++17", "-ffp-contract=off", "-munsafe-fp-atomics"};
        const hiprtcResult r = hiprtcCompileProgram(prog, 5, opts);
        if (r != HIPRTC_SUCCESS) {
            size_t n = 0; (void)hiprtcGetProgramLogSize(prog, &n);
            std::string log(n + 1, '\0');
            if (n) (void)hiprtcGetProgramLog(prog, &log[0]);
            (void)hiprtcDestroyProgram(&prog);
            if (std::getenv("SDQLPY_AMD_JIT_DUMP")) std::fprintf(stderr, "---- specialised source ----\n%s\n", source.c_str());
            return fail(ctx, SDQH_ERR_DEVICE, std::string("hiprtc: ") + hiprtcGetErrorString(r) + "\n" + log.substr(0, 4000));
        }
        size_t n = 0; (void)hiprtcGetCodeSize(prog, &n);
        code.resize(n);
        (void)hiprtcGetCode(prog, &code[0]);
        (void)hiprtcDestroyProgram(&prog);
        ++J.compiled;
        if (const char* rdir = std::getenv("SDQLPY_AMD_JIT_RECIPES")) {
            char rn[32]; std::snprintf(rn, sizeof(rn), "%016llx", (unsigned long long)fnv1a(source));
            (void)mkdir(rdir, 0777);
            std::ofstream rf(std::string(rdir) + "/" + rn + ".hip", std::ios::binary);
            rf << source;
        }
        const std::string tmp = path + ".tmp." + std::to_string((long)getpid());
        { std::ofstream f(tmp, std::ios::binary); f.write(code.data(), (std::streamsize)code.size()); }
        (void)std::rename(tmp.c_str(), path.c_str());
    }
    if (ctx->compile_only) return fail(ctx, SDQH_ERR_DEVICE, "compile-only context: kernel specialised (" + std::to_string(code.size()) + " bytes of gfx950 code), not run");
    hipModule_t mod;
    if (hipModuleLoadData(&mod, code.data()) != hipSuccess) { (void)hipGetLastError(); return fail(ctx, SDQH_ERR_DEVICE, "hipModuleLoadData failed for a specialised kernel"); }
    hipFunction_t f;
    if (hipModuleGetFunction(&f, mod, entry.c_str()) != hipSuccess) { (void)hipGetLastError(); return fail(ctx, SDQH_ERR_DEVICE, "specialised kernel has no entry point"); }
    J.kernels[key] = f;
    *fn = f;
    return SDQH_OK;
}

template <class SA> struct Packed { XArgs a; SA s; int64_t nrows; int64_t seg_rows; int32_t nseg; };

int fill_xargs(sdqh_ctx* ctx, const XInfo& x, XArgs* a, int32_t* flags, int64_t key_lo, int64_t key_hi) {
    std::memset(a, 0, sizeof(*a));
    for (int c = 0; c < x.ncols; ++c) { a->col[c] = x.cols[c]->data; a->width[c] = x.cols[c]->width; a->ncol[c] = (((x.narrow_mask | x.gather32) >> c) & 1u) ? x.cols[c]->narrow : nullptr; }
    for (int t = 0; t < x.ntabs; ++t) {
        if (int rc = index_ensure(ctx, x.tabs[t])) return rc;
        a->tab[t] = x.tabs[t]->dev;
    }
    if (x.tight) for (int c = 0; c < x.ncols; ++c) a->dlo[c] = x.dlo[c];
    if (x.tight) for (int c = 0; c < x.ncols; ++c) if (x.enc[c] == ENC_D8) a->dcol[c] = x.cols[c]->delta8;
    if (x.tight) for (int c = 0; c < x.ncols; ++c) if (x.enc[c] >= ENC_C16) { a->code[c] = x.cols[c]->code; a->dict[c] = static_cast<const int64_t*>(x.cols[c]->dict); a->ndict[c] = x.cols[c]->ndict; }
    std::memcpy(a->cc, x.cc, sizeof(x.cc[0]) * (size_t)x.ncc);
    std::memcpy(a->ci, x.ci, sizeof(x.ci[0]) * (size_t)x.nci);
    std::memcpy(a->cf, x.cf, sizeof(x.cf[0]) * (size_t)x.ncf);
    std::memcpy(a->spool, x.spool, sizeof(uint32_t) * (size_t)x.nstr);
    a->flags = flags; a->key_lo = key_lo; a->key_hi = key_hi;
    if (x.driven && x.driven_col >= 0 && x.cols[x.driven_col]->run_index_state == 1) {
        const sdqh_column* kc = x.cols[x.driven_col];
        a->run_index = static_cast<const uint32_t*>(kc->run_index); a->run_lo = kc->mn; a->run_hi = kc->mx; a->driven_ratio = ctx->opt_x_driven;
    }
    return SDQH_OK;
}

struct Geometry { unsigned grid; int64_t seg_rows; int nseg; };
Geometry geometry_tight(sdqh_ctx* ctx, int64_t nrows, int resident, bool pipelined = false) {
    const int64_t steps = std::max<int64_t>(1, nrows / ((int64_t)XT_ROWS * (pipelined ? 1 : 2)));
    return Geometry{(unsigned)std::min<int64_t>(steps, (int64_t)ctx->num_cu * resident), 0, 0};
}
Geometry geometry(sdqh_ctx* ctx, int64_t nrows, bool direct, int waves_per_cu, bool tight = false, bool tiled = false) {
    Geometry g{1, 0, 0};
    static const bool no_tiles = getenv("SDQLPY_AMD_X_NOTILED") != nullptr;
    if (tiled && tight && !direct && !no_tiles && nrows < ((int64_t)1 << 31) && nrows >= (int64_t)X8_STEP * X8_U) {
        if (ctx->opt_x_waves > 0) waves_per_cu = ctx->opt_x_waves;
        const int64_t steps = nrows / ((int64_t)X8_STEP * X8_U);
        g.seg_rows = 0;
        g.nseg = (int)std::max<int64_t>(1, std::min<int64_t>(steps, (int64_t)ctx->num_cu * waves_per_cu));
        g.grid = (unsigned)((g.nseg + TPB / WAVE - 1) / (TPB / WAVE));
        return g;
    }
    if (direct) {
        const int64_t tiles = ((nrows + TILE_ROWS - 1) / TILE_ROWS + SDQH_TILE_CHUNK - 1) / SDQH_TILE_CHUNK;
        g.grid = (unsigned)std::max<int64_t>(1, std::min<int64_t>(tiles, (int64_t)ctx->num_cu * ctx->opt_resident_stream));
        return g;
    }
    const int64_t gran = tight ? (int64_t)X8_STEP * X8_U : (int64_t)WAVE * ROWS_PER_LOAD * X_LB;
    if (ctx->opt_x_waves > 0) waves_per_cu = ctx->opt_x_waves;
    const int64_t target = (int64_t)ctx->num_cu * waves_per_cu;
    int64_t seg_rows = (nrows + target - 1) / target;
    seg_rows = std::max<int64_t>(gran, (seg_rows + gran - 1) / gran * gran);
    g.seg_rows = seg_rows;
    g.nseg = (int)std::max<int64_t>(1, (nrows + seg_rows - 1) / seg_rows);
    g.grid = (unsigned)((g.nseg + TPB / WAVE - 1) / (TPB / WAVE));
    return g;
}

template <class SA>
int launch(sdqh_ctx* ctx, hipFunction_t fn, const char* name, const XArgs& a, const SA& sa, int64_t nrows, const Geometry& g, unsigned lds_bytes = 0) {
    Packed<SA> pk;
    std::memset(&pk, 0, sizeof(pk));
    pk.a = a; pk.s = sa; pk.nrows = nrows; pk.seg_rows = g.seg_rows; pk.nseg = g.nseg;
    size_t size = sizeof(pk);
    void* config[] = {HIP_LAUNCH_PARAM_BUFFER_POINTER, &pk, HIP_LAUNCH_PARAM_BUFFER_SIZE, &size, HIP_LAUNCH_PARAM_END};
    KernelScope ks(ctx, name);
    HIP_TRY(ctx, hipModuleLaunchKernel(fn, g.grid, 1, 1, TPB, 1, 1, lds_bytes, ctx->stream, nullptr, config));
    return SDQH_OK;
}

int64_t model_stream_bytes(const XInfo& x, int64_t nrows, bool regs_all) {
    int64_t per_row = 0, per_8rows = 0;
    for (int c = 0; c < x.ncols; ++c) {
        bool streamed = regs_all;
        if (!streamed) for (int sc : x.scols) streamed = streamed || sc == c;
        if (!streamed || x.cols[c]->dtype == SDQH_STR) continue;
        if (x.tight && x.enc[c] == ENC_D8) { per_8rows += 12; continue; }
        if (x.tight) per_row += x.enc[c] == ENC_C8 ? 1 : x.enc[c] == ENC_C16 ? 2 : x.enc[c] == ENC_N32 ? 4 : 8;
        else per_row += ((x.narrow_mask >> c) & 1u) ? 4 : 8;
    }
    int64_t bytes = per_row * nrows + per_8rows * ((nrows + 7) / 8);
    auto bitmap = [&](const sdqh_table* t) { if (t && t->dev.bm && t->dev.bm_hi >= t->dev.bm_lo) bytes += (int64_t)(((uint64_t)(t->dev.bm_hi - t->dev.bm_lo) >> t->dev.bm_shift) / 8 + 4); };
    if (x.vstage) for (int l = 0; l < x.nlk; ++l) bitmap(x.tabs[x.tab_of[x.lk_op[l]]]);
    else if (!regs_all && x.prefilter_op >= 0) bitmap(x.tabs[x.tab_of[x.prefilter_op]]);
    return bytes;
}

int read_flags(sdqh_ctx* ctx, const int32_t* d_flags, int* out) {
    HIP_TRY(ctx, hipMemcpyAsync(ctx->result_host, d_flags, 4, hipMemcpyDeviceToHost, ctx->stream));
    if (int rc = sync_stream(ctx)) return rc;
    *out = *static_cast<const int*>(ctx->result_host);
    return SDQH_OK;
// ... 491 lines not shown
```

sdqlpy_amd/jit_recipes/135b4eca74295a68.hip:

```cpp
#include "sdqh_xkernels.hpp"
using namespace sdqh;
struct P {
    static constexpr int NS = 1, NV = 1, NSC = 0, NSOP = 0, ND = 0;
    struct Regs { uint32_t c0[8]; };
    __device__ __forceinline__ static void load_dicts(const XArgs& a, int64_t (*tab)[256]) {
    }
    template <bool TAIL> __device__ __forceinline__ static void sload(const XArgs& a, int64_t r, int64_t nrows, Regs& s) {
        xt_load<4, TAIL>(a.ncol[0], r, nrows, s.c0);
    }
    __device__ __forceinline__ static bool stest(const XArgs& a, const Regs& s, const int64_t (*tab)[256], const int i) {
        bool p = true;
        const int64_t v0 = (int64_t)xt_i32(s.c0, i);
        p = p && x_may_hit(a.tab[0], v0, false);
        return p;
    }
    __device__ __forceinline__ static bool spre(const XArgs& a, const Regs& s, const int64_t (*tab)[256], const int i, uint32_t& widx, uint32_t& bit) {
        bool p = true;
        const int64_t v0 = (int64_t)xt_i32(s.c0, i);
        const bool in = (v0 >= a.tab[0].bm_lo) & (v0 <= a.tab[0].bm_hi);
        p = p & in;
        const uint64_t off = in ? (uint64_t)(v0 - a.tab[0].bm_lo) : 0ull;
        widx = (uint32_t)(off >> 5); bit = (uint32_t)off & 31u;
        return p;
    }
    static constexpr bool PREF32 = true, PWIN = false;
    __device__ __forceinline__ static bool spre32(const XArgs& a, const Regs& s, const int64_t (*tab)[256], const int i, uint32_t& off) {
        bool p = true;
        const int64_t v0 = (int64_t)xt_i32(s.c0, i);
        const uint32_t o32 = (uint32_t)((int32_t)v0 - (int32_t)a.tab[0].bm_lo);
        const bool in = o32 <= (uint32_t)(a.tab[0].bm_hi - a.tab[0].bm_lo);
        p = p & in;
        off = in ? o32 : 0u;
        return p;
    }
    __device__ __forceinline__ static const uint32_t* sbitmap(const XArgs& a) { return x_prefilter_bitmap(a.tab[0], false); }
    template <int H> __device__ __forceinline__ static bool eval_regs(const XArgs& a, const Pair<int64_t> (&s)[1], int64_t r, XOut<NV>& o) {
        return false;
    }
    __device__ __forceinline__ static bool eval_row(const XArgs& a, int64_t r, const int64_t (&sres)[1], XOut<NV>& o) {
        int64_t v0 = (int64_t)static_cast<const int32_t*>(a.ncol[0])[r];
        int64_t v2 = (int64_t)static_cast<const int32_t*>(a.ncol[1])[r];
        x_pin(v0, v2);
        const uint32_t e1 = x_lookup_l<0x80000082u>(a.tab[0], v0, false);
        const bool v1 = (e1 != NO_ROW);
        int64_t v3 = x_field(a.tab[0], 1, e1);
        x_pin(v3);
        if (!v1) return false;
        const bool b4 = false || false || v2 < 0 || v2 > 0xFFFFFFFFll || v3 < 0 || v3 > 0xFFFFFFFFll;
        const int64_t v4 = (int64_t)(((uint64_t)v2 << 32) | ((uint64_t)v3 & 0xFFFFFFFFull));
        const uint32_t e5 = x_lookup_l<0x80000052u>(a.tab[1], v4, b4);
        const bool v5 = (e5 != NO_ROW);
        if (!v5) return false;
        int64_t v6 = x_field(a.tab[0], 0, e1);
        double v7 = narrow_decode(static_cast<const int32_t*>(a.ncol[2])[r]);
        double v9 = narrow_decode(static_cast<const int32_t*>(a.ncol[3])[r]);
        x_pin(v6, v7, v9);
        o.key = v6; o.bad = false;
        const double v8 = a.cf[0];
        const double v10 = (v8 - v9);
        const double v11 = (v7 * v10);
        o.val[0] = x_bits(v11);
        o.ent = NO_ROW;
        return true;
    }
};
extern "C" __global__ __launch_bounds__(256) void xk_group_tight(XArgs a, XGroup<P::NV>::Args s, int64_t nrows, int64_t seg_rows, int nseg) {
    x_queue8<P, XGroup, false>(a, s, nrows, seg_rows, nseg);
}
```

sdqlpy_amd/jit_recipes/7691e0f2c096ce65.hip:

```cpp
#include "sdqh_xkernels.hpp"
using namespace sdqh;
struct P {
    static constexpr int NS = 1, NV = 1, NSC = 0, NSOP = 0, ND = 0;
    struct Regs { uint32_t c0[16]; };
    __device__ __forceinline__ static void load_dicts(const XArgs& a, int64_t (*tab)[256]) {
    }
    template <bool TAIL> __device__ __forceinline__ static void sload(const XArgs& a, int64_t r, int64_t nrows, Regs& s) {
        xt_load<8, TAIL>(a.col[0], r, nrows, s.c0);
    }
    __device__ __forceinline__ static bool stest(const XArgs& a, const Regs& s, const int64_t (*tab)[256], const int i) {
        bool p = true;
        const int64_t v0 = xt_i64(s.c0, i);
        p = p && x_may_hit(a.tab[0], v0, false);
        return p;
    }
    __device__ __forceinline__ static bool spre(const XArgs& a, const Regs& s, const int64_t (*tab)[256], const int i, uint32_t& widx, uint32_t& bit) {
        bool p = true;
        const int64_t v0 = xt_i64(s.c0, i);
        const bool in = (v0 >= a.tab[0].bm_lo) & (v0 <= a.tab[0].bm_hi);
        p = p & in;
        const uint64_t off = p ? (uint64_t)(v0 - a.tab[0].bm_lo) : 0ull;
        widx = (uint32_t)(off >> 5); bit = (uint32_t)off & 31u;
        return p;
    }
    static constexpr bool PREF32 = false, PWIN = false;
    __device__ __forceinline__ static bool spre32(const XArgs& a, const Regs& s, const int64_t (*tab)[256], const int i, uint32_t& off) {
        off = 0; return false;
    }
    __device__ __forceinline__ static const uint32_t* sbitmap(const XArgs& a) { return x_prefilter_bitmap(a.tab[0], false); }
    template <int H> __device__ __forceinline__ static bool eval_regs(const XArgs& a, const Pair<int64_t> (&s)[1], int64_t r, XOut<NV>& o) {
        return false;
    }
    __device__ __forceinline__ static bool eval_row(const XArgs& a, int64_t r, const int64_t (&sres)[1], XOut<NV>& o) {
        int64_t v0 = static_cast<const int64_t*>(a.col[0])[r];
        int64_t v2 = static_cast<const int64_t*>(a.col[1])[r];
        x_pin(v0, v2);
        const uint32_t e1 = x_lookup_l<0x80000043u>(a.tab[0], v0, false);
        const bool v1 = (e1 != NO_ROW);
        int64_t v3 = x_field(a.tab[0], 1, e1);
        x_pin(v3);
        if (!v1) return false;
        const bool b4 = false || false || v2 < 0 || v2 > 0xFFFFFFFFll || v3 < 0 || v3 > 0xFFFFFFFFll;
        const int64_t v4 = (int64_t)(((uint64_t)v2 << 32) | ((uint64_t)v3 & 0xFFFFFFFFull));
        const uint32_t e5 = x_lookup_l<0x80000052u>(a.tab[1], v4, b4);
        const bool v5 = (e5 != NO_ROW);
        if (!v5) return false;
        int64_t v6 = x_field(a.tab[0], 0, e1);
        double v7 = static_cast<const double*>(a.col[2])[r];
        double v9 = static_cast<const double*>(a.col[3])[r];
        x_pin(v6, v7, v9);
        o.key = v6; o.bad = false;
        const double v8 = a.cf[0];
        const double v10 = (v8 - v9);
        const double v11 = (v7 * v10);
        o.val[0] = x_bits(v11);
        o.ent = NO_ROW;
        return true;
    }
};
extern "C" __global__ __launch_bounds__(256) void xk_group_tight(XArgs a, XGroup<P::NV>::Args s, int64_t nrows, int64_t seg_rows, int nseg) {
    x_queue8<P, XGroup, false>(a, s, nrows, seg_rows, nseg);
}
```

sdqlpy_amd/jit_recipes/8ce169e172faea2f.hip:

```cpp
#include "sdqh_xkernels.hpp"
using namespace sdqh;
struct P {
    static constexpr int NS = 1, NV = 1, NSC = 0, NSOP = 0, ND = 0;
    struct Regs { uint32_t c0[8]; };
    __device__ __forceinline__ static void load_dicts(const XArgs& a, int64_t (*tab)[256]) {
    }
    template <bool TAIL> __device__ __forceinline__ static void sload(const XArgs& a, int64_t r, int64_t nrows, Regs& s) {
        xt_load<4, TAIL>(a.ncol[0], r, nrows, s.c0);
    }
    __device__ __forceinline__ static bool stest(const XArgs& a, const Regs& s, const int64_t (*tab)[256], const int i) {
        bool p = true;
        const int64_t v0 = (int64_t)xt_i32(s.c0, i);
        p = p && x_may_hit(a.tab[0], v0, false);
        return p;
    }
    __device__ __forceinline__ static bool spre(const XArgs& a, const Regs& s, const int64_t (*tab)[256], const int i, uint32_t& widx, uint32_t& bit) {
        bool p = true;
        const int64_t v0 = (int64_t)xt_i32(s.c0, i);
        const bool in = (v0 >= a.tab[0].bm_lo) & (v0 <= a.tab[0].bm_hi);
        p = p & in;
        const uint64_t off = in ? (uint64_t)(v0 - a.tab[0].bm_lo) : 0ull;
        widx = (uint32_t)(off >> 5); bit = (uint32_t)off & 31u;
        return p;
    }
    static constexpr bool PREF32 = true, PWIN = false;
    __device__ __forceinline__ static bool spre32(const XArgs& a, const Regs& s, const int64_t (*tab)[256], const int i, uint32_t& off) {
        bool p = true;
        const int64_t v0 = (int64_t)xt_i32(s.c0, i);
        const uint32_t o32 = (uint32_t)((int32_t)v0 - (int32_t)a.tab[0].bm_lo);
        const bool in = o32 <= (uint32_t)(a.tab[0].bm_hi - a.tab[0].bm_lo);
        p = p & in;
        off = in ? o32 : 0u;
        return p;
    }
    __device__ __forceinline__ static const uint32_t* sbitmap(const XArgs& a) { return x_prefilter_bitmap(a.tab[0], false); }
    static constexpr bool DRIVEN = true;
    __device__ __forceinline__ static const DevTable& dtab(const XArgs& a) { return a.tab[0]; }
    template <int H> __device__ __forceinline__ static bool eval_regs(const XArgs& a, const Pair<int64_t> (&s)[1], int64_t r, XOut<NV>& o) {
        return false;
    }
    __device__ __forceinline__ static bool eval_row(const XArgs& a, int64_t r, const int64_t (&sres)[1], XOut<NV>& o) {
        int64_t v0 = (int64_t)static_cast<const int32_t*>(a.ncol[0])[r];
        int64_t v2 = (int64_t)static_cast<const int32_t*>(a.ncol[1])[r];
        x_pin(v0, v2);
        const uint32_t e1 = x_lookup_l<0x80000043u>(a.tab[0], v0, false);
        const bool v1 = (e1 != NO_ROW);
        int64_t v3 = x_field(a.tab[0], 1, e1);
        x_pin(v3);
        if (!v1) return false;
        const bool b4 = false || false || v2 < 0 || v2 > 0xFFFFFFFFll || v3 < 0 || v3 > 0xFFFFFFFFll;
        const int64_t v4 = (int64_t)(((uint64_t)v2 << 32) | ((uint64_t)v3 & 0xFFFFFFFFull));
        const uint32_t e5 = x_lookup_l<0x80000052u>(a.tab[1], v4, b4);
        const bool v5 = (e5 != NO_ROW);
        if (!v5) return false;
        int64_t v6 = x_field(a.tab[0], 0, e1);
        double v7 = narrow_decode(static_cast<const int32_t*>(a.ncol[2])[r]);
        double v9 = narrow_decode(static_cast<const int32_t*>(a.ncol[3])[r]);
        x_pin(v6, v7, v9);
        o.key = v6; o.bad = false;
        const double v8 = a.cf[0];
        const double v10 = (v8 - v9);
        const double v11 = (v7 * v10);
        o.val[0] = x_bits(v11);
        o.ent = NO_ROW;
        return true;
    }
};
extern "C" __global__ __launch_bounds__(256) void xk_group_tight(XArgs a, XGroup<P::NV>::Args s, int64_t nrows, int64_t seg_rows, int nseg) {
    x_queue8<P, XGroup, false>(a, s, nrows, seg_rows, nseg);
}
```

sdqlpy_amd/jit_recipes/c1cdd91cbcf9195e.hip:

```cpp
#include "sdqh_xkernels.hpp"
using namespace sdqh;
struct P {
    static constexpr int NS = 1, NV = 1, NSC = 0, NSOP = 0, ND = 0;
    struct Regs { uint32_t c0[8]; };
    __device__ __forceinline__ static void load_dicts(const XArgs& a, int64_t (*tab)[256]) {
    }
    template <bool TAIL> __device__ __forceinline__ static void sload(const XArgs& a, int64_t r, int64_t nrows, Regs& s) {
        xt_load<4, TAIL>(a.ncol[0], r, nrows, s.c0);
    }
    __device__ __forceinline__ static bool stest(const XArgs& a, const Regs& s, const int64_t (*tab)[256], const int i) {
        bool p = true;
        const int64_t v0 = (int64_t)xt_i32(s.c0, i);
        p = p && x_may_hit(a.tab[0], v0, false);
        return p;
    }
    __device__ __forceinline__ static bool spre(const XArgs& a, const Regs& s, const int64_t (*tab)[256], const int i, uint32_t& widx, uint32_t& bit) {
        bool p = true;
        const int64_t v0 = (int64_t)xt_i32(s.c0, i);
        const bool in = (v0 >= a.tab[0].bm_lo) & (v0 <= a.tab[0].bm_hi);
        p = p & in;
        const uint64_t off = in ? (uint64_t)(v0 - a.tab[0].bm_lo) : 0ull;
        widx = (uint32_t)(off >> 5); bit = (uint32_t)off & 31u;
        return p;
    }
    static constexpr bool PREF32 = true, PWIN = false;
    __device__ __forceinline__ static bool spre32(const XArgs& a, const Regs& s, const int64_t (*tab)[256], const int i, uint32_t& off) {
        bool p = true;
        const int64_t v0 = (int64_t)xt_i32(s.c0, i);
        const uint32_t o32 = (uint32_t)((int32_t)v0 - (int32_t)a.tab[0].bm_lo);
        const bool in = o32 <= (uint32_t)(a.tab[0].bm_hi - a.tab[0].bm_lo);
        p = p & in;
        off = in ? o32 : 0u;
        return p;
    }
    __device__ __forceinline__ static const uint32_t* sbitmap(const XArgs& a) { return x_prefilter_bitmap(a.tab[0], false); }
    static constexpr bool DRIVEN = true;
    __device__ __forceinline__ static const DevTable& dtab(const XArgs& a) { return a.tab[0]; }
    template <int H> __device__ __forceinline__ static bool eval_regs(const XArgs& a, const Pair<int64_t> (&s)[1], int64_t r, XOut<NV>& o) {
        return false;
    }
    __device__ __forceinline__ static bool eval_row(const XArgs& a, int64_t r, const int64_t (&sres)[1], XOut<NV>& o) {
        int64_t v0 = (int64_t)static_cast<const int32_t*>(a.ncol[0])[r];
        int64_t v2 = (int64_t)static_cast<const int32_t*>(a.ncol[1])[r];
        x_pin(v0, v2);
        const uint32_t e1 = x_lookup_l<0x80000082u>(a.tab[0], v0, false);
        const bool v1 = (e1 != NO_ROW);
        int64_t v3 = x_field(a.tab[0], 1, e1);
        x_pin(v3);
        if (!v1) return false;
        const bool b4 = false || false || v2 < 0 || v2 > 0xFFFFFFFFll || v3 < 0 || v3 > 0xFFFFFFFFll;
        const int64_t v4 = (int64_t)(((uint64_t)v2 << 32) | ((uint64_t)v3 & 0xFFFFFFFFull));
        const uint32_t e5 = x_lookup_l<0x80000052u>(a.tab[1], v4, b4);
        const bool v5 = (e5 != NO_ROW);
        if (!v5) return false;
        int64_t v6 = x_field(a.tab[0], 0, e1);
        double v7 = narrow_decode(static_cast<const int32_t*>(a.ncol[2])[r]);
        double v9 = narrow_decode(static_cast<const int32_t*>(a.ncol[3])[r]);
        x_pin(v6, v7, v9);
        o.key = v6; o.bad = false;
        const double v8 = a.cf[0];
        const double v10 = (v8 - v9);
        const double v11 = (v7 * v10);
        o.val[0] = x_bits(v11);
        o.ent = NO_ROW;
        return true;
    }
};
extern "C" __global__ __launch_bounds__(256) void xk_group_tight(XArgs a, XGroup<P::NV>::Args s, int64_t nrows, int64_t seg_rows, int nseg) {
    x_queue8<P, XGroup, false>(a, s, nrows, seg_rows, nseg);
}
```

Before: 446.4 billion rows/s.

## Use workgroup-scope handoff in single-block index build and skip index for membership-only tables

When the index build runs in one workgroup, the rank step now writes the header counters directly instead of through atomics. It also swaps the device-wide threadfence for workgroup-scoped release/acquire fences around the barrier. Separately, a table used only for membership lookups (no field reads, not the probe or prefilter table) gets a bitmap-only layout, so its dense index build is skipped and the JIT kernel specialises for that layout. This cuts fence and atomic cost and removes per-table index work. The risk is correctness if the single-workgroup assumption fails, which an assert guards, or if a later consumer needs the index.

```diff
diff --git a/sdqlpy_amd/csrc/sdqh_hip.hip b/sdqlpy_amd/csrc/sdqh_hip.hip
--- a/sdqlpy_amd/csrc/sdqh_hip.hip
+++ b/sdqlpy_amd/csrc/sdqh_hip.hip
@@ -1,6 +1,7 @@
 #include <hip/hip_runtime.h>
 
 #include <algorithm>
+#include <cassert>
 #include <atomic>
 #include <chrono>
 #include <cmath>
@@ -682,6 +683,8 @@
     else if (n == "grouped_index" && (value == 0 || value == 1)) ctx->opt_grouped_index = (int)value;
     else if (n == "grouped_pairs" && (value == 0 || value == 1)) ctx->opt_grouped_pairs = (int)value;
     else if (n == "index_inline" && (value == 0 || value == 1)) ctx->opt_index_inline = (int)value;
+    else if (n == "wg_handoff" && (value == 0 || value == 1)) ctx->opt_wg_handoff = (int)value;
+    else if (n == "x_member" && (value == 0 || value == 1)) ctx->opt_x_member = (int)value;
     else if (n == "groupby_regs" && (value == 0 || value == 4 || value == 8)) ctx->opt_groupby_regs = (int)value;
     else if (n == "hash_filter" && (value == 0 || value == 1)) ctx->opt_hash_filter = (int)value;
     else if (n == "pack_ordered" && (value == 0 || value == 1)) ctx->opt_pack_ordered = (int)value;
@@ -1100,7 +1103,7 @@
         if (!wprefix || !dense) return fail(ctx, SDQH_ERR_NOMEM, "table index: out of device memory");
         tb->dev.wprefix = wprefix; tb->dev.dense_ref = dense;
         if (nblocks == 1 && seg_grid == 1 && tb->refs_prefilled && ctx->opt_fuse_small) {
-            LAUNCH(ctx, "k_index_small", k_index_small, 1u, tb->bm, tb->nwords, wprefix, tb->stage, tb->dev, tb->span);
+            LAUNCH(ctx, "k_index_small", k_index_small, 1u, tb->bm, tb->nwords, wprefix, tb->stage, tb->dev, tb->span, ctx->opt_wg_handoff);
             if (tb->span) tb->dev.dense_arr = tb->span;
             hipError_t es = hipGetLastError();
             if (es != hipSuccess) return fail(ctx, SDQH_ERR_DEVICE, std::string("table index launch: ") + hipGetErrorString(es));
@@ -2019,9 +2022,10 @@
             uint32_t* wprefix = static_cast<uint32_t*>(table_alloc(ctx, tb, tb->nwords * 4 + 64));
             if (wprefix) {
                 tb->dev.wprefix = wprefix;
-                ix.t = tb->dev; ix.wprefix = wprefix; ix.span = tb->span; ix.nwords = tb->nwords; ix.on = 1;
+                ix.t = tb->dev; ix.wprefix = wprefix; ix.span = tb->span; ix.nwords = tb->nwords; ix.on = 1; ix.wg = ctx->opt_wg_handoff;
             }
         }
+        assert(!ix.on || seg_grid == 1);
         hipError_t e;
         with_scan_filter(f, [&](auto FC) {
             using FCT = decltype(FC);
diff --git a/sdqlpy_amd/csrc/sdqh_host.hpp b/sdqlpy_amd/csrc/sdqh_host.hpp
--- a/sdqlpy_amd/csrc/sdqh_host.hpp
+++ b/sdqlpy_amd/csrc/sdqh_host.hpp
@@ -99,6 +99,8 @@
     int opt_grouped_index = 1;
     int opt_grouped_pairs = 1;
     int opt_index_inline = 1;
+    int opt_wg_handoff = 1;
+    int opt_x_member = 1;
     int opt_lane_int = 1;
     int opt_lane_resident = 2;
     int opt_window = 0;
diff --git a/sdqlpy_amd/csrc/sdqh_kernels.hpp b/sdqlpy_amd/csrc/sdqh_kernels.hpp
--- a/sdqlpy_amd/csrc/sdqh_kernels.hpp
+++ b/sdqlpy_amd/csrc/sdqh_kernels.hpp
@@ -1312,6 +1312,7 @@
     for (uint64_t i = (uint64_t)blockIdx.x * TPB + threadIdx.x; i < cap / 2; i += (uint64_t)gridDim.x * TPB) k2[i] = empty;
 }
 
+template <bool ONE = false>
 __device__ __forceinline__ void rank_words_body(const uint32_t* __restrict__ bm, uint64_t nwords, uint32_t* __restrict__ wprefix,
                                                 const uint32_t* __restrict__ seg_count, int nseg, TableHeader* __restrict__ hdr) {
     __shared__ uint32_t s_wave[TPB / WAVE];
@@ -1348,14 +1349,23 @@
         excl[r] = running + before + incl - mine;
         running += total;
     }
-    uint32_t stg = 0;
-    for (int i = blockIdx.x * TPB + threadIdx.x; i < nseg; i += gridDim.x * TPB) stg += seg_count[i];
-#pragma unroll
-    for (int off = WAVE / 2; off > 0; off >>= 1) stg += __shfl_down(stg, off, WAVE);
-    if (lane == 0 && stg) atomicAdd(reinterpret_cast<unsigned long long*>(&hdr->staged), (unsigned long long)stg);
-    if (threadIdx.x == 0) s_base = running ? (uint32_t)atomicAdd(reinterpret_cast<unsigned long long*>(&hdr->distinct), (unsigned long long)running) : 0u;
-    __syncthreads();
-    const uint32_t base = s_base;
+    uint32_t base = 0;
+    if constexpr (ONE) {
+        if (threadIdx.x == 0) {
+            uint64_t stg = 0;
+            for (int i = 0; i < nseg; ++i) stg += seg_count[i];
+            hdr->staged = stg; hdr->distinct = running;
+        }
+    } else {
+        uint32_t stg = 0;
+        for (int i = blockIdx.x * TPB + threadIdx.x; i < nseg; i += gridDim.x * TPB) stg += seg_count[i];
+#pragma unroll
+        for (int off = WAVE / 2; off > 0; off >>= 1) stg += __shfl_down(stg, off, WAVE);
+        if (lane == 0 && stg) atomicAdd(reinterpret_cast<unsigned long long*>(&hdr->staged), (unsigned long long)stg);
+        if (threadIdx.x == 0) s_base = running ? (uint32_t)atomicAdd(reinterpret_cast<unsigned long long*>(&hdr->distinct), (unsigned long long)running) : 0u;
+        __syncthreads();
+        base = s_base;
+    }
 #pragma unroll
     for (int r = 0; r < ROWS; ++r) {
         const uint64_t qi = q0 + (uint64_t)r * TPB + threadIdx.x;
@@ -1416,11 +1426,24 @@
     }
 }
 SDQH_KERNEL __launch_bounds__(TPB) void k_insert_direct(DevStage st, DevTable t, uint32_t* __restrict__ span) { insert_direct_body(st, t, span); }
-SDQH_KERNEL __launch_bounds__(TPB) void k_index_small(const uint32_t* __restrict__ bm, uint64_t nwords, uint32_t* __restrict__ wprefix, DevStage st, DevTable t, uint32_t* __restrict__ span) {
-    rank_words_body(bm, nwords, wprefix, st.seg_count, st.nseg, t.hdr);
-    __threadfence();
-    __syncthreads();
+__device__ __forceinline__ void workgroup_handoff() {
+    __builtin_amdgcn_fence(__ATOMIC_RELEASE, "workgroup");
+    __syncthreads();
+    __builtin_amdgcn_fence(__ATOMIC_ACQUIRE, "workgroup");
+}
+__device__ __forceinline__ void index_one_workgroup(const uint32_t* bm, uint64_t nwords, uint32_t* wprefix, const DevStage& st, const DevTable& t, uint32_t* span, bool wg) {
+    if (wg) {
+        rank_words_body<true>(bm, nwords, wprefix, st.seg_count, st.nseg, t.hdr);
+        workgroup_handoff();
+    } else {
+        rank_words_body(bm, nwords, wprefix, st.seg_count, st.nseg, t.hdr);
+        __threadfence();
+        __syncthreads();
+    }
     insert_direct_body(st, t, span);
+}
+SDQH_KERNEL __launch_bounds__(TPB) void k_index_small(const uint32_t* __restrict__ bm, uint64_t nwords, uint32_t* __restrict__ wprefix, DevStage st, DevTable t, uint32_t* __restrict__ span, int wg) {
+    index_one_workgroup(bm, nwords, wprefix, st, t, span, wg != 0);
 }
 SDQH_KERNEL __launch_bounds__(TPB) void k_index_medium(const uint32_t* __restrict__ bm, uint32_t nwords, uint32_t* __restrict__ wprefix, DevStage st, DevTable t, uint32_t* __restrict__ span) {
     __shared__ uint32_t s_word[RANK_BLOCK_WORDS], s_pre[RANK_BLOCK_WORDS];
@@ -2243,7 +2266,7 @@
     DevSource pay[SDQH_MAX_PAYLOAD];
 };
 
-struct DevIndexInline { DevTable t; uint32_t* wprefix; uint32_t* span; uint64_t nwords; int32_t on, _pad; };
+struct DevIndexInline { DevTable t; uint32_t* wprefix; uint32_t* span; uint64_t nwords; int32_t on, wg; };
 
 template <class FC, bool NW>
 __device__ __forceinline__ void build_lookup_segment(const DevFilter& f, const DevLookups& L, const DevBuildSpec& spec, const DevStage& st, int64_t nrows, int* __restrict__ flags,
@@ -2370,12 +2393,8 @@
     const int seg = blockIdx.x * (TPB / WAVE) + threadIdx.x / WAVE;
     if (seg < st.nseg) build_lookup_segment<FC, NW>(f, L, spec, st, nrows, flags, nkey0, npred0, s_row[threadIdx.x / WAVE], seg);
     if (ix.on) {
-        __threadfence();
-        __syncthreads();
-        rank_words_body(st.bm, ix.nwords, ix.wprefix, st.seg_count, st.nseg, st.hdr);
-        __threadfence();
-        __syncthreads();
-        insert_direct_body(st, ix.t, ix.span);
+        if (ix.wg) workgroup_handoff(); else { __threadfence(); __syncthreads(); }
+        index_one_workgroup(st.bm, ix.nwords, ix.wprefix, st, ix.t, ix.span, ix.wg != 0);
     }
 }
 
diff --git a/sdqlpy_amd/csrc/sdqh_x.hip b/sdqlpy_amd/csrc/sdqh_x.hip
--- a/sdqlpy_amd/csrc/sdqh_x.hip
+++ b/sdqlpy_amd/csrc/sdqh_x.hip
@@ -1189,12 +1189,33 @@
 
 int specialise(sdqh_ctx* ctx, const std::string& source, const std::string& entry, hipFunction_t* fn);
 
+static bool layouts_off() { static const bool off = std::getenv("SDQLPY_AMD_X_NOLAYOUT") != nullptr; return off; }
+
+uint32_t member_layout(const sdqh_ctx* ctx, const XInfo& x, int t) {
+    if (!ctx->opt_x_member || ctx->compile_only || layouts_off() || x.vstage) return 0u;
+    const sdqh_table* tb = x.tabs[t];
+    if (tb->bitmap_only || !tb->dev.bm || tb->dev.bm_shift != 0 || tb->dev.grp_first) return 0u;
+    if (x.probe_op >= 0 && x.tab_of[x.probe_op] == t) return 0u;
+    if (x.prefilter_op >= 0 && x.tab_of[x.prefilter_op] == t) return 0u;
+    for (int k = 0; k < x.p->nops; ++k) {
+        const sdqh_xop& o = x.p->ops[k];
+        if ((o.code == SDQH_X_FIELD || o.code == SDQH_X_ACC) && x.tab_of[o.a] == t) return 0u;
+    }
+    const uint32_t l = x_layout_of(tb->dev, true);
+    return (l & XL_KNOWN) ? (l & (XL_KNOWN | XL_BM | XL_LIN | XL_BITMAP_ONLY)) : 0u;
+}
+
 int kernel_for(sdqh_ctx* ctx, const XInfo& x, Sink sink, bool direct, hipFunction_t* fn) {
     JitState& J = jit();
-    static const bool no_layouts = std::getenv("SDQLPY_AMD_X_NOLAYOUT") != nullptr;
+    const bool no_layouts = layouts_off();
     uint64_t lay_hash = 0;
     for (int t = 0; t < x.ntabs; ++t) {
         if (ctx->compile_only) { x.lay[t] = 0u; continue; }
+        if (const uint32_t ml = member_layout(ctx, x, t)) {
+            x.lay[t] = ml;
+            lay_hash = (lay_hash ^ x.lay[t]) * 0x9E3779B97F4A7C15ull + (uint64_t)t;
+            continue;
+        }
         if (int rc = index_ensure(ctx, x.tabs[t])) return rc;
         x.lay[t] = no_layouts ? 0u : x_layout_of(x.tabs[t]->dev, x.tabs[t]->bitmap_only);
         lay_hash = (lay_hash ^ x.lay[t]) * 0x9E3779B97F4A7C15ull + (uint64_t)t;
@@ -1283,7 +1304,7 @@
     std::memset(a, 0, sizeof(*a));
     for (int c = 0; c < x.ncols; ++c) { a->col[c] = x.cols[c]->data; a->width[c] = x.cols[c]->width; a->ncol[c] = (((x.narrow_mask | x.gather32) >> c) & 1u) ? x.cols[c]->narrow : nullptr; }
     for (int t = 0; t < x.ntabs; ++t) {
-        if (int rc = index_ensure(ctx, x.tabs[t])) return rc;
+        if (!member_layout(ctx, x, t)) { if (int rc = index_ensure(ctx, x.tabs[t])) return rc; }
         a->tab[t] = x.tabs[t]->dev;
     }
     if (x.tight) for (int c = 0; c < x.ncols; ++c) a->dlo[c] = x.dlo[c];
diff --git a/sdqlpy_amd/jit_recipes/135b4eca74295a68.hip b/sdqlpy_amd/jit_recipes/135b4eca74295a68.hip
--- a/sdqlpy_amd/jit_recipes/135b4eca74295a68.hip
+++ /dev/null
@@ -1,69 +0,0 @@
-#include "sdqh_xkernels.hpp"
-using namespace sdqh;
-struct P {
-    static constexpr int NS = 1, NV = 1, NSC = 0, NSOP = 0, ND = 0;
-    struct Regs { uint32_t c0[8]; };
-    __device__ __forceinline__ static void load_dicts(const XArgs& a, int64_t (*tab)[256]) {
-    }
-    template <bool TAIL> __device__ __forceinline__ static void sload(const XArgs& a, int64_t r, int64_t nrows, Regs& s) {
-        xt_load<4, TAIL>(a.ncol[0], r, nrows, s.c0);
-    }
-    __device__ __forceinline__ static bool stest(const XArgs& a, const Regs& s, const int64_t (*tab)[256], const int i) {
-        bool p = true;
-        const int64_t v0 = (int64_t)xt_i32(s.c0, i);
-        p = p && x_may_hit(a.tab[0], v0, false);
-        return p;
-    }
-    __device__ __forceinline__ static bool spre(const XArgs& a, const Regs& s, const int64_t (*tab)[256], const int i, uint32_t& widx, uint32_t& bit) {
-        bool p = true;
-        const int64_t v0 = (int64_t)xt_i32(s.c0, i);
-        const bool in = (v0 >= a.tab[0].bm_lo) & (v0 <= a.tab[0].bm_hi);
-        p = p & in;
-        const uint64_t off = in ? (uint64_t)(v0 - a.tab[0].bm_lo) : 0ull;
-        widx = (uint32_t)(off >> 5); bit = (uint32_t)off & 31u;
-        return p;
-    }
-    static constexpr bool PREF32 = true, PWIN = false;
-    __device__ __forceinline__ static bool spre32(const XArgs& a, const Regs& s, const int64_t (*tab)[256], const int i, uint32_t& off) {
-        bool p = true;
-        const int64_t v0 = (int64_t)xt_i32(s.c0, i);
-        const uint32_t o32 = (uint32_t)((int32_t)v0 - (int32_t)a.tab[0].bm_lo);
-        const bool in = o32 <= (uint32_t)(a.tab[0].bm_hi - a.tab[0].bm_lo);
-        p = p & in;
-        off = in ? o32 : 0u;
-        return p;
-    }
-    __device__ __forceinline__ static const uint32_t* sbitmap(const XArgs& a) { return x_prefilter_bitmap(a.tab[0], false); }
-    template <int H> __device__ __forceinline__ static bool eval_regs(const XArgs& a, const Pair<int64_t> (&s)[1], int64_t r, XOut<NV>& o) {
-        return false;
-    }
-    __device__ __forceinline__ static bool eval_row(const XArgs& a, int64_t r, const int64_t (&sres)[1], XOut<NV>& o) {
-        int64_t v0 = (int64_t)static_cast<const int32_t*>(a.ncol[0])[r];
-        int64_t v2 = (int64_t)static_cast<const int32_t*>(a.ncol[1])[r];
-        x_pin(v0, v2);
-        const uint32_t e1 = x_lookup_l<0x80000082u>(a.tab[0], v0, false);
-        const bool v1 = (e1 != NO_ROW);
-        int64_t v3 = x_field(a.tab[0], 1, e1);
-        x_pin(v3);
-        if (!v1) return false;
-        const bool b4 = false || false || v2 < 0 || v2 > 0xFFFFFFFFll || v3 < 0 || v3 > 0xFFFFFFFFll;
-        const int64_t v4 = (int64_t)(((uint64_t)v2 << 32) | ((uint64_t)v3 & 0xFFFFFFFFull));
-        const uint32_t e5 = x_lookup_l<0x80000052u>(a.tab[1], v4, b4);
-        const bool v5 = (e5 != NO_ROW);
-        if (!v5) return false;
-        int64_t v6 = x_field(a.tab[0], 0, e1);
-        double v7 = narrow_decode(static_cast<const int32_t*>(a.ncol[2])[r]);
-        double v9 = narrow_decode(static_cast<const int32_t*>(a.ncol[3])[r]);
-        x_pin(v6, v7, v9);
-        o.key = v6; o.bad = false;
-        const double v8 = a.cf[0];
-        const double v10 = (v8 - v9);
-        const double v11 = (v7 * v10);
-        o.val[0] = x_bits(v11);
-        o.ent = NO_ROW;
-        return true;
-    }
-};
-extern "C" __global__ __launch_bounds__(256) void xk_group_tight(XArgs a, XGroup<P::NV>::Args s, int64_t nrows, int64_t seg_rows, int nseg) {
-    x_queue8<P, XGroup, false>(a, s, nrows, seg_rows, nseg);
-}
diff --git a/sdqlpy_amd/jit_recipes/2db6b92236c0bb09.hip b/sdqlpy_amd/jit_recipes/2db6b92236c0bb09.hip
--- /dev/null
+++ b/sdqlpy_amd/jit_recipes/2db6b92236c0bb09.hip
@@ -0,0 +1,71 @@
+#include "sdqh_xkernels.hpp"
+using namespace sdqh;
+struct P {
+    static constexpr int NS = 1, NV = 1, NSC = 0, NSOP = 0, ND = 0;
+    struct Regs { uint32_t c0[8]; };
+    __device__ __forceinline__ static void load_dicts(const XArgs& a, int64_t (*tab)[256]) {
+    }
+    template <bool TAIL> __device__ __forceinline__ static void sload(const XArgs& a, int64_t r, int64_t nrows, Regs& s) {
+        xt_load<4, TAIL>(a.ncol[0], r, nrows, s.c0);
+    }
+    __device__ __forceinline__ static bool stest(const XArgs& a, const Regs& s, const int64_t (*tab)[256], const int i) {
+        bool p = true;
+        const int64_t v0 = (int64_t)xt_i32(s.c0, i);
+        p = p && x_may_hit(a.tab[0], v0, false);
+        return p;
+    }
+    __device__ __forceinline__ static bool spre(const XArgs& a, const Regs& s, const int64_t (*tab)[256], const int i, uint32_t& widx, uint32_t& bit) {
+        bool p = true;
+        const int64_t v0 = (int64_t)xt_i32(s.c0, i);
+        const bool in = (v0 >= a.tab[0].bm_lo) & (v0 <= a.tab[0].bm_hi);
+        p = p & in;
+        const uint64_t off = in ? (uint64_t)(v0 - a.tab[0].bm_lo) : 0ull;
+        widx = (uint32_t)(off >> 5); bit = (uint32_t)off & 31u;
+        return p;
+    }
+    static constexpr bool PREF32 = true, PWIN = false;
+    __device__ __forceinline__ static bool spre32(const XArgs& a, const Regs& s, const int64_t (*tab)[256], const int i, uint32_t& off) {
+        bool p = true;
+        const int64_t v0 = (int64_t)xt_i32(s.c0, i);
+        const uint32_t o32 = (uint32_t)((int32_t)v0 - (int32_t)a.tab[0].bm_lo);
+        const bool in = o32 <= (uint32_t)(a.tab[0].bm_hi - a.tab[0].bm_lo);
+        p = p & in;
+        off = in ? o32 : 0u;
+        return p;
+    }
+    __device__ __forceinline__ static const uint32_t* sbitmap(const XArgs& a) { return x_prefilter_bitmap(a.tab[0], false); }
+    static constexpr bool DRIVEN = true;
+    __device__ __forceinline__ static const DevTable& dtab(const XArgs& a) { return a.tab[0]; }
+    template <int H> __device__ __forceinline__ static bool eval_regs(const XArgs& a, const Pair<int64_t> (&s)[1], int64_t r, XOut<NV>& o) {
+        return false;
+    }
+    __device__ __forceinline__ static bool eval_row(const XArgs& a, int64_t r, const int64_t (&sres)[1], XOut<NV>& o) {
+        int64_t v0 = (int64_t)static_cast<const int32_t*>(a.ncol[0])[r];
+        int64_t v2 = (int64_t)static_cast<const int32_t*>(a.ncol[1])[r];
+        x_pin(v0, v2);
+        const uint32_t e1 = x_lookup_l<0x80000082u>(a.tab[0], v0, false);
+        const bool v1 = (e1 != NO_ROW);
+        int64_t v3 = x_field(a.tab[0], 1, e1);
+        x_pin(v3);
+        if (!v1) return false;
+        const bool b4 = false || false || v2 < 0 || v2 > 0xFFFFFFFFll || v3 < 0 || v3 > 0xFFFFFFFFll;
+        const int64_t v4 = (int64_t)(((uint64_t)v2 << 32) | ((uint64_t)v3 & 0xFFFFFFFFull));
+        const uint32_t e5 = x_lookup_l<0x8000001au>(a.tab[1], v4, b4);
+        const bool v5 = (e5 != NO_ROW);
+        if (!v5) return false;
+        int64_t v6 = x_field(a.tab[0], 0, e1);
+        double v7 = narrow_decode(static_cast<const int32_t*>(a.ncol[2])[r]);
+        double v9 = narrow_decode(static_cast<const int32_t*>(a.ncol[3])[r]);
+        x_pin(v6, v7, v9);
+        o.key = v6; o.bad = false;
+        const double v8 = a.cf[0];
+        const double v10 = (v8 - v9);
+        const double v11 = (v7 * v10);
+        o.val[0] = x_bits(v11);
+        o.ent = NO_ROW;
+        return true;
+    }
+};
+extern "C" __global__ __launch_bounds__(256) void xk_group_tight(XArgs a, XGroup<P::NV>::Args s, int64_t nrows, int64_t seg_rows, int nseg) {
+    x_queue8<P, XGroup, false>(a, s, nrows, seg_rows, nseg);
+}
diff --git a/sdqlpy_amd/jit_recipes/322b20264620f167.hip b/sdqlpy_amd/jit_recipes/322b20264620f167.hip
--- /dev/null
+++ b/sdqlpy_amd/jit_recipes/322b20264620f167.hip
@@ -0,0 +1,69 @@
+#include "sdqh_xkernels.hpp"
+using namespace sdqh;
+struct P {
+    static constexpr int NS = 1, NV = 1, NSC = 0, NSOP = 0, ND = 0;
+    struct Regs { uint32_t c0[8]; };
+    __device__ __forceinline__ static void load_dicts(const XArgs& a, int64_t (*tab)[256]) {
+    }
+    template <bool TAIL> __device__ __forceinline__ static void sload(const XArgs& a, int64_t r, int64_t nrows, Regs& s) {
+        xt_load<4, TAIL>(a.ncol[0], r, nrows, s.c0);
+    }
+    __device__ __forceinline__ static bool stest(const XArgs& a, const Regs& s, const int64_t (*tab)[256], const int i) {
+        bool p = true;
+        const int64_t v0 = (int64_t)xt_i32(s.c0, i);
+        p = p && x_may_hit(a.tab[0], v0, false);
+        return p;
+    }
+    __device__ __forceinline__ static bool spre(const XArgs& a, const Regs& s, const int64_t (*tab)[256], const int i, uint32_t& widx, uint32_t& bit) {
+        bool p = true;
+        const int64_t v0 = (int64_t)xt_i32(s.c0, i);
+        const bool in = (v0 >= a.tab[0].bm_lo) & (v0 <= a.tab[0].bm_hi);
+        p = p & in;
+        const uint64_t off = in ? (uint64_t)(v0 - a.tab[0].bm_lo) : 0ull;
+        widx = (uint32_t)(off >> 5); bit = (uint32_t)off & 31u;
+        return p;
+    }
+    static constexpr bool PREF32 = true, PWIN = false;
+    __device__ __forceinline__ static bool spre32(const XArgs& a, const Regs& s, const int64_t (*tab)[256], const int i, uint32_t& off) {
+        bool p = true;
+        const int64_t v0 = (int64_t)xt_i32(s.c0, i);
+        const uint32_t o32 = (uint32_t)((int32_t)v0 - (int32_t)a.tab[0].bm_lo);
+        const bool in = o32 <= (uint32_t)(a.tab[0].bm_hi - a.tab[0].bm_lo);
+        p = p & in;
+        off = in ? o32 : 0u;
+        return p;
+    }
+    __device__ __forceinline__ static const uint32_t* sbitmap(const XArgs& a) { return x_prefilter_bitmap(a.tab[0], false); }
+    template <int H> __device__ __forceinline__ static bool eval_regs(const XArgs& a, const Pair<int64_t> (&s)[1], int64_t r, XOut<NV>& o) {
+        return false;
+    }
+    __device__ __forceinline__ static bool eval_row(const XArgs& a, int64_t r, const int64_t (&sres)[1], XOut<NV>& o) {
+        int64_t v0 = (int64_t)static_cast<const int32_t*>(a.ncol[0])[r];
+        int64_t v2 = (int64_t)static_cast<const int32_t*>(a.ncol[1])[r];
+        x_pin(v0, v2);
+        const uint32_t e1 = x_lookup_l<0x80000082u>(a.tab[0], v0, false);
+        const bool v1 = (e1 != NO_ROW);
+        int64_t v3 = x_field(a.tab[0], 1, e1);
+        x_pin(v3);
+        if (!v1) return false;
+        const bool b4 = false || false || v2 < 0 || v2 > 0xFFFFFFFFll || v3 < 0 || v3 > 0xFFFFFFFFll;
+        const int64_t v4 = (int64_t)(((uint64_t)v2 << 32) | ((uint64_t)v3 & 0xFFFFFFFFull));
+        const uint32_t e5 = x_lookup_l<0x8000001au>(a.tab[1], v4, b4);
+        const bool v5 = (e5 != NO_ROW);
+        if (!v5) return false;
+        int64_t v6 = x_field(a.tab[0], 0, e1);
+        double v7 = narrow_decode(static_cast<const int32_t*>(a.ncol[2])[r]);
+        double v9 = narrow_decode(static_cast<const int32_t*>(a.ncol[3])[r]);
+        x_pin(v6, v7, v9);
+        o.key = v6; o.bad = false;
+        const double v8 = a.cf[0];
+        const double v10 = (v8 - v9);
+        const double v11 = (v7 * v10);
+        o.val[0] = x_bits(v11);
+        o.ent = NO_ROW;
+        return true;
+    }
+};
+extern "C" __global__ __launch_bounds__(256) void xk_group_tight(XArgs a, XGroup<P::NV>::Args s, int64_t nrows, int64_t seg_rows, int nseg) {
+    x_queue8<P, XGroup, false>(a, s, nrows, seg_rows, nseg);
+}
diff --git a/sdqlpy_amd/jit_recipes/5915eb07aed6e9d0.hip b/sdqlpy_amd/jit_recipes/5915eb07aed6e9d0.hip
--- /dev/null
+++ b/sdqlpy_amd/jit_recipes/5915eb07aed6e9d0.hip
@@ -0,0 +1,71 @@
+#include "sdqh_xkernels.hpp"
+using namespace sdqh;
+struct P {
+    static constexpr int NS = 1, NV = 1, NSC = 0, NSOP = 0, ND = 0;
+    struct Regs { uint32_t c0[8]; };
+    __device__ __forceinline__ static void load_dicts(const XArgs& a, int64_t (*tab)[256]) {
+    }
+    template <bool TAIL> __device__ __forceinline__ static void sload(const XArgs& a, int64_t r, int64_t nrows, Regs& s) {
+        xt_load<4, TAIL>(a.ncol[0], r, nrows, s.c0);
+    }
+    __device__ __forceinline__ static bool stest(const XArgs& a, const Regs& s, const int64_t (*tab)[256], const int i) {
+        bool p = true;
+        const int64_t v0 = (int64_t)xt_i32(s.c0, i);
+        p = p && x_may_hit(a.tab[0], v0, false);
+        return p;
+    }
+    __device__ __forceinline__ static bool spre(const XArgs& a, const Regs& s, const int64_t (*tab)[256], const int i, uint32_t& widx, uint32_t& bit) {
+        bool p = true;
+        const int64_t v0 = (int64_t)xt_i32(s.c0, i);
+        const bool in = (v0 >= a.tab[0].bm_lo) & (v0 <= a.tab[0].bm_hi);
+        p = p & in;
+        const uint64_t off = in ? (uint64_t)(v0 - a.tab[0].bm_lo) : 0ull;
+        widx = (uint32_t)(off >> 5); bit = (uint32_t)off & 31u;
+        return p;
+    }
+    static constexpr bool PREF32 = true, PWIN = false;
+    __device__ __forceinline__ static bool spre32(const XArgs& a, const Regs& s, const int64_t (*tab)[256], const int i, uint32_t& off) {
+        bool p = true;
+        const int64_t v0 = (int64_t)xt_i32(s.c0, i);
+        const uint32_t o32 = (uint32_t)((int32_t)v0 - (int32_t)a.tab[0].bm_lo);
+        const bool in = o32 <= (uint32_t)(a.tab[0].bm_hi - a.tab[0].bm_lo);
+        p = p & in;
+        off = in ? o32 : 0u;
+        return p;
+    }
+    __device__ __forceinline__ static const uint32_t* sbitmap(const XArgs& a) { return x_prefilter_bitmap(a.tab[0], false); }
+    static constexpr bool DRIVEN = true;
+    __device__ __forceinline__ static const DevTable& dtab(const XArgs& a) { return a.tab[0]; }
+    template <int H> __device__ __forceinline__ static bool eval_regs(const XArgs& a, const Pair<int64_t> (&s)[1], int64_t r, XOut<NV>& o) {
+        return false;
+    }
+    __device__ __forceinline__ static bool eval_row(const XArgs& a, int64_t r, const int64_t (&sres)[1], XOut<NV>& o) {
+        int64_t v0 = (int64_t)static_cast<const int32_t*>(a.ncol[0])[r];
+        int64_t v2 = (int64_t)static_cast<const int32_t*>(a.ncol[1])[r];
+        x_pin(v0, v2);
+        const uint32_t e1 = x_lookup_l<0x80000043u>(a.tab[0], v0, false);
+        const bool v1 = (e1 != NO_ROW);
+        int64_t v3 = x_field(a.tab[0], 1, e1);
+        x_pin(v3);
+        if (!v1) return false;
+        const bool b4 = false || false || v2 < 0 || v2 > 0xFFFFFFFFll || v3 < 0 || v3 > 0xFFFFFFFFll;
+        const int64_t v4 = (int64_t)(((uint64_t)v2 << 32) | ((uint64_t)v3 & 0xFFFFFFFFull));
+        const uint32_t e5 = x_lookup_l<0x8000001au>(a.tab[1], v4, b4);
+        const bool v5 = (e5 != NO_ROW);
+        if (!v5) return false;
+        int64_t v6 = x_field(a.tab[0], 0, e1);
+        double v7 = narrow_decode(static_cast<const int32_t*>(a.ncol[2])[r]);
+        double v9 = narrow_decode(static_cast<const int32_t*>(a.ncol[3])[r]);
+        x_pin(v6, v7, v9);
+        o.key = v6; o.bad = false;
+        const double v8 = a.cf[0];
+        const double v10 = (v8 - v9);
+        const double v11 = (v7 * v10);
+        o.val[0] = x_bits(v11);
+        o.ent = NO_ROW;
+        return true;
+    }
+};
+extern "C" __global__ __launch_bounds__(256) void xk_group_tight(XArgs a, XGroup<P::NV>::Args s, int64_t nrows, int64_t seg_rows, int nseg) {
+    x_queue8<P, XGroup, false>(a, s, nrows, seg_rows, nseg);
+}
diff --git a/sdqlpy_amd/jit_recipes/7691e0f2c096ce65.hip b/sdqlpy_amd/jit_recipes/7691e0f2c096ce65.hip
--- a/sdqlpy_amd/jit_recipes/7691e0f2c096ce65.hip
+++ /dev/null
@@ -1,63 +0,0 @@
-#include "sdqh_xkernels.hpp"
-using namespace sdqh;
-struct P {
-    static constexpr int NS = 1, NV = 1, NSC = 0, NSOP = 0, ND = 0;
-    struct Regs { uint32_t c0[16]; };
-    __device__ __forceinline__ static void load_dicts(const XArgs& a, int64_t (*tab)[256]) {
-    }
-    template <bool TAIL> __device__ __forceinline__ static void sload(const XArgs& a, int64_t r, int64_t nrows, Regs& s) {
-        xt_load<8, TAIL>(a.col[0], r, nrows, s.c0);
-    }
-    __device__ __forceinline__ static bool stest(const XArgs& a, const Regs& s, const int64_t (*tab)[256], const int i) {
-        bool p = true;
-        const int64_t v0 = xt_i64(s.c0, i);
-        p = p && x_may_hit(a.tab[0], v0, false);
-        return p;
-    }
-    __device__ __forceinline__ static bool spre(const XArgs& a, const Regs& s, const int64_t (*tab)[256], const int i, uint32_t& widx, uint32_t& bit) {
-        bool p = true;
-        const int64_t v0 = xt_i64(s.c0, i);
-        const bool in = (v0 >= a.tab[0].bm_lo) & (v0 <= a.tab[0].bm_hi);
-        p = p & in;
-        const uint64_t off = p ? (uint64_t)(v0 - a.tab[0].bm_lo) : 0ull;
-        widx = (uint32_t)(off >> 5); bit = (uint32_t)off & 31u;
-        return p;
-    }
-    static constexpr bool PREF32 = false, PWIN = false;
-    __device__ __forceinline__ static bool spre32(const XArgs& a, const Regs& s, const int64_t (*tab)[256], const int i, uint32_t& off) {
-        off = 0; return false;
-    }
-    __device__ __forceinline__ static const uint32_t* sbitmap(const XArgs& a) { return x_prefilter_bitmap(a.tab[0], false); }
-    template <int H> __device__ __forceinline__ static bool eval_regs(const XArgs& a, const Pair<int64_t> (&s)[1], int64_t r, XOut<NV>& o) {
-        return false;
-    }
-    __device__ __forceinline__ static bool eval_row(const XArgs& a, int64_t r, const int64_t (&sres)[1], XOut<NV>& o) {
-        int64_t v0 = static_cast<const int64_t*>(a.col[0])[r];
-        int64_t v2 = static_cast<const int64_t*>(a.col[1])[r];
-        x_pin(v0, v2);
-        const uint32_t e1 = x_lookup_l<0x80000043u>(a.tab[0], v0, false);
-        const bool v1 = (e1 != NO_ROW);
-        int64_t v3 = x_field(a.tab[0], 1, e1);
-        x_pin(v3);
-        if (!v1) return false;
-        const bool b4 = false || false || v2 < 0 || v2 > 0xFFFFFFFFll || v3 < 0 || v3 > 0xFFFFFFFFll;
-        const int64_t v4 = (int64_t)(((uint64_t)v2 << 32) | ((uint64_t)v3 & 0xFFFFFFFFull));
-        const uint32_t e5 = x_lookup_l<0x80000052u>(a.tab[1], v4, b4);
-        const bool v5 = (e5 != NO_ROW);
-        if (!v5) return false;
-        int64_t v6 = x_field(a.tab[0], 0, e1);
-        double v7 = static_cast<const double*>(a.col[2])[r];
-        double v9 = static_cast<const double*>(a.col[3])[r];
-        x_pin(v6, v7, v9);
-        o.key = v6; o.bad = false;
-        const double v8 = a.cf[0];
-        const double v10 = (v8 - v9);
-        const double v11 = (v7 * v10);
-        o.val[0] = x_bits(v11);
-        o.ent = NO_ROW;
-        return true;
-    }
-};
-extern "C" __global__ __launch_bounds__(256) void xk_group_tight(XArgs a, XGroup<P::NV>::Args s, int64_t nrows, int64_t seg_rows, int nseg) {
-    x_queue8<P, XGroup, false>(a, s, nrows, seg_rows, nseg);
-}
diff --git a/sdqlpy_amd/jit_recipes/8ce169e172faea2f.hip b/sdqlpy_amd/jit_recipes/8ce169e172faea2f.hip
--- a/sdqlpy_amd/jit_recipes/8ce169e172faea2f.hip
+++ /dev/null
@@ -1,71 +0,0 @@
-#include "sdqh_xkernels.hpp"
-using namespace sdqh;
-struct P {
-    static constexpr int NS = 1, NV = 1, NSC = 0, NSOP = 0, ND = 0;
-    struct Regs { uint32_t c0[8]; };
-    __device__ __forceinline__ static void load_dicts(const XArgs& a, int64_t (*tab)[256]) {
-    }
-    template <bool TAIL> __device__ __forceinline__ static void sload(const XArgs& a, int64_t r, int64_t nrows, Regs& s) {
-        xt_load<4, TAIL>(a.ncol[0], r, nrows, s.c0);
-    }
-    __device__ __forceinline__ static bool stest(const XArgs& a, const Regs& s, const int64_t (*tab)[256], const int i) {
-        bool p = true;
-        const int64_t v0 = (int64_t)xt_i32(s.c0, i);
-        p = p && x_may_hit(a.tab[0], v0, false);
-        return p;
-    }
-    __device__ __forceinline__ static bool spre(const XArgs& a, const Regs& s, const int64_t (*tab)[256], const int i, uint32_t& widx, uint32_t& bit) {
-        bool p = true;
-        const int64_t v0 = (int64_t)xt_i32(s.c0, i);
-        const bool in = (v0 >= a.tab[0].bm_lo) & (v0 <= a.tab[0].bm_hi);
-        p = p & in;
-        const uint64_t off = in ? (uint64_t)(v0 - a.tab[0].bm_lo) : 0ull;
-        widx = (uint32_t)(off >> 5); bit = (uint32_t)off & 31u;
-        return p;
-    }
-    static constexpr bool PREF32 = true, PWIN = false;
-    __device__ __forceinline__ static bool spre32(const XArgs& a, const Regs& s, const int64_t (*tab)[256], const int i, uint32_t& off) {
-        bool p = true;
-        const int64_t v0 = (int64_t)xt_i32(s.c0, i);
-        const uint32_t o32 = (uint32_t)((int32_t)v0 - (int32_t)a.tab[0].bm_lo);
-        const bool in = o32 <= (uint32_t)(a.tab[0].bm_hi - a.tab[0].bm_lo);
-        p = p & in;
-        off = in ? o32 : 0u;
-        return p;
-    }
-    __device__ __forceinline__ static const uint32_t* sbitmap(const XArgs& a) { return x_prefilter_bitmap(a.tab[0], false); }
-    static constexpr bool DRIVEN = true;
-    __device__ __forceinline__ static const DevTable& dtab(const XArgs& a) { return a.tab[0]; }
-    template <int H> __device__ __forceinline__ static bool eval_regs(const XArgs& a, const Pair<int64_t> (&s)[1], int64_t r, XOut<NV>& o) {
-        return false;
-    }
-    __device__ __forceinline__ static bool eval_row(const XArgs& a, int64_t r, const int64_t (&sres)[1], XOut<NV>& o) {
-        int64_t v0 = (int64_t)static_cast<const int32_t*>(a.ncol[0])[r];
-        int64_t v2 = (int64_t)static_cast<const int32_t*>(a.ncol[1])[r];
-        x_pin(v0, v2);
-        const uint32_t e1 = x_lookup_l<0x80000043u>(a.tab[0], v0, false);
-        const bool v1 = (e1 != NO_ROW);
-        int64_t v3 = x_field(a.tab[0], 1, e1);
-        x_pin(v3);
-        if (!v1) return false;
-        const bool b4 = false || false || v2 < 0 || v2 > 0xFFFFFFFFll || v3 < 0 || v3 > 0xFFFFFFFFll;
-        const int64_t v4 = (int64_t)(((uint64_t)v2 << 32) | ((uint64_t)v3 & 0xFFFFFFFFull));
-        const uint32_t e5 = x_lookup_l<0x80000052u>(a.tab[1], v4, b4);
-        const bool v5 = (e5 != NO_ROW);
-        if (!v5) return false;
-        int64_t v6 = x_field(a.tab[0], 0, e1);
-        double v7 = narrow_decode(static_cast<const int32_t*>(a.ncol[2])[r]);
-        double v9 = narrow_decode(static_cast<const int32_t*>(a.ncol[3])[r]);
-        x_pin(v6, v7, v9);
-        o.key = v6; o.bad = false;
-        const double v8 = a.cf[0];
-        const double v10 = (v8 - v9);
-        const double v11 = (v7 * v10);
-        o.val[0] = x_bits(v11);
-        o.ent = NO_ROW;
-        return true;
-    }
-};
-extern "C" __global__ __launch_bounds__(256) void xk_group_tight(XArgs a, XGroup<P::NV>::Args s, int64_t nrows, int64_t seg_rows, int nseg) {
-    x_queue8<P, XGroup, false>(a, s, nrows, seg_rows, nseg);
-}
diff --git a/sdqlpy_amd/jit_recipes/c1cdd91cbcf9195e.hip b/sdqlpy_amd/jit_recipes/c1cdd91cbcf9195e.hip
--- a/sdqlpy_amd/jit_recipes/c1cdd91cbcf9195e.hip
+++ /dev/null
@@ -1,71 +0,0 @@
-#include "sdqh_xkernels.hpp"
-using namespace sdqh;
-struct P {
-    static constexpr int NS = 1, NV = 1, NSC = 0, NSOP = 0, ND = 0;
-    struct Regs { uint32_t c0[8]; };
-    __device__ __forceinline__ static void load_dicts(const XArgs& a, int64_t (*tab)[256]) {
-    }
-    template <bool TAIL> __device__ __forceinline__ static void sload(const XArgs& a, int64_t r, int64_t nrows, Regs& s) {
-        xt_load<4, TAIL>(a.ncol[0], r, nrows, s.c0);
-    }
-    __device__ __forceinline__ static bool stest(const XArgs& a, const Regs& s, const int64_t (*tab)[256], const int i) {
-        bool p = true;
-        const int64_t v0 = (int64_t)xt_i32(s.c0, i);
-        p = p && x_may_hit(a.tab[0], v0, false);
-        return p;
-    }
-    __device__ __forceinline__ static bool spre(const XArgs& a, const Regs& s, const int64_t (*tab)[256], const int i, uint32_t& widx, uint32_t& bit) {
-        bool p = true;
-        const int64_t v0 = (int64_t)xt_i32(s.c0, i);
-        const bool in = (v0 >= a.tab[0].bm_lo) & (v0 <= a.tab[0].bm_hi);
-        p = p & in;
-        const uint64_t off = in ? (uint64_t)(v0 - a.tab[0].bm_lo) : 0ull;
-        widx = (uint32_t)(off >> 5); bit = (uint32_t)off & 31u;
-        return p;
-    }
-    static constexpr bool PREF32 = true, PWIN = false;
-    __device__ __forceinline__ static bool spre32(const XArgs& a, const Regs& s, const int64_t (*tab)[256], const int i, uint32_t& off) {
-        bool p = true;
-        const int64_t v0 = (int64_t)xt_i32(s.c0, i);
-        const uint32_t o32 = (uint32_t)((int32_t)v0 - (int32_t)a.tab[0].bm_lo);
-        const bool in = o32 <= (uint32_t)(a.tab[0].bm_hi - a.tab[0].bm_lo);
-        p = p & in;
-        off = in ? o32 : 0u;
-        return p;
-    }
-    __device__ __forceinline__ static const uint32_t* sbitmap(const XArgs& a) { return x_prefilter_bitmap(a.tab[0], false); }
-    static constexpr bool DRIVEN = true;
-    __device__ __forceinline__ static const DevTable& dtab(const XArgs& a) { return a.tab[0]; }
-    template <int H> __device__ __forceinline__ static bool eval_regs(const XArgs& a, const Pair<int64_t> (&s)[1], int64_t r, XOut<NV>& o) {
-        return false;
-    }
-    __device__ __forceinline__ static bool eval_row(const XArgs& a, int64_t r, const int64_t (&sres)[1], XOut<NV>& o) {
-        int64_t v0 = (int64_t)static_cast<const int32_t*>(a.ncol[0])[r];
-        int64_t v2 = (int64_t)static_cast<const int32_t*>(a.ncol[1])[r];
-        x_pin(v0, v2);
-        const uint32_t e1 = x_lookup_l<0x80000082u>(a.tab[0], v0, false);
-        const bool v1 = (e1 != NO_ROW);
-        int64_t v3 = x_field(a.tab[0], 1, e1);
-        x_pin(v3);
-        if (!v1) return false;
-        const bool b4 = false || false || v2 < 0 || v2 > 0xFFFFFFFFll || v3 < 0 || v3 > 0xFFFFFFFFll;
-        const int64_t v4 = (int64_t)(((uint64_t)v2 << 32) | ((uint64_t)v3 & 0xFFFFFFFFull));
-        const uint32_t e5 = x_lookup_l<0x80000052u>(a.tab[1], v4, b4);
-        const bool v5 = (e5 != NO_ROW);
-        if (!v5) return false;
-        int64_t v6 = x_field(a.tab[0], 0, e1);
-        double v7 = narrow_decode(static_cast<const int32_t*>(a.ncol[2])[r]);
-        double v9 = narrow_decode(static_cast<const int32_t*>(a.ncol[3])[r]);
-        x_pin(v6, v7, v9);
-        o.key = v6; o.bad = false;
-        const double v8 = a.cf[0];
-        const double v10 = (v8 - v9);
-        const double v11 = (v7 * v10);
-        o.val[0] = x_bits(v11);
-        o.ent = NO_ROW;
-        return true;
-    }
-};
-extern "C" __global__ __launch_bounds__(256) void xk_group_tight(XArgs a, XGroup<P::NV>::Args s, int64_t nrows, int64_t seg_rows, int nseg) {
-    x_queue8<P, XGroup, false>(a, s, nrows, seg_rows, nseg);
-}
diff --git a/sdqlpy_amd/jit_recipes/e935e9c26f2f3456.hip b/sdqlpy_amd/jit_recipes/e935e9c26f2f3456.hip
--- /dev/null
+++ b/sdqlpy_amd/jit_recipes/e935e9c26f2f3456.hip
@@ -0,0 +1,63 @@
+#include "sdqh_xkernels.hpp"
+using namespace sdqh;
+struct P {
+    static constexpr int NS = 1, NV = 1, NSC = 0, NSOP = 0, ND = 0;
+    struct Regs { uint32_t c0[16]; };
+    __device__ __forceinline__ static void load_dicts(const XArgs& a, int64_t (*tab)[256]) {
+    }
+    template <bool TAIL> __device__ __forceinline__ static void sload(const XArgs& a, int64_t r, int64_t nrows, Regs& s) {
+        xt_load<8, TAIL>(a.col[0], r, nrows, s.c0);
+    }
+    __device__ __forceinline__ static bool stest(const XArgs& a, const Regs& s, const int64_t (*tab)[256], const int i) {
+        bool p = true;
+        const int64_t v0 = xt_i64(s.c0, i);
+        p = p && x_may_hit(a.tab[0], v0, false);
+        return p;
+    }
+    __device__ __forceinline__ static bool spre(const XArgs& a, const Regs& s, const int64_t (*tab)[256], const int i, uint32_t& widx, uint32_t& bit) {
+        bool p = true;
+        const int64_t v0 = xt_i64(s.c0, i);
+        const bool in = (v0 >= a.tab[0].bm_lo) & (v0 <= a.tab[0].bm_hi);
+        p = p & in;
+        const uint64_t off = p ? (uint64_t)(v0 - a.tab[0].bm_lo) : 0ull;
+        widx = (uint32_t)(off >> 5); bit = (uint32_t)off & 31u;
+        return p;
+    }
+    static constexpr bool PREF32 = false, PWIN = false;
+    __device__ __forceinline__ static bool spre32(const XArgs& a, const Regs& s, const int64_t (*tab)[256], const int i, uint32_t& off) {
+        off = 0; return false;
+    }
+    __device__ __forceinline__ static const uint32_t* sbitmap(const XArgs& a) { return x_prefilter_bitmap(a.tab[0], false); }
+    template <int H> __device__ __forceinline__ static bool eval_regs(const XArgs& a, const Pair<int64_t> (&s)[1], int64_t r, XOut<NV>& o) {
+        return false;
+    }
+    __device__ __forceinline__ static bool eval_row(const XArgs& a, int64_t r, const int64_t (&sres)[1], XOut<NV>& o) {
+        int64_t v0 = static_cast<const int64_t*>(a.col[0])[r];
+        int64_t v2 = static_cast<const int64_t*>(a.col[1])[r];
+        x_pin(v0, v2);
+        const uint32_t e1 = x_lookup_l<0x80000043u>(a.tab[0], v0, false);
+        const bool v1 = (e1 != NO_ROW);
+        int64_t v3 = x_field(a.tab[0], 1, e1);
+        x_pin(v3);
+        if (!v1) return false;
+        const bool b4 = false || false || v2 < 0 || v2 > 0xFFFFFFFFll || v3 < 0 || v3 > 0xFFFFFFFFll;
+        const int64_t v4 = (int64_t)(((uint64_t)v2 << 32) | ((uint64_t)v3 & 0xFFFFFFFFull));
+        const uint32_t e5 = x_lookup_l<0x8000001au>(a.tab[1], v4, b4);
+        const bool v5 = (e5 != NO_ROW);
+        if (!v5) return false;
+        int64_t v6 = x_field(a.tab[0], 0, e1);
+        double v7 = static_cast<const double*>(a.col[2])[r];
+        double v9 = static_cast<const double*>(a.col[3])[r];
+        x_pin(v6, v7, v9);
+        o.key = v6; o.bad = false;
+        const double v8 = a.cf[0];
+        const double v10 = (v8 - v9);
+        const double v11 = (v7 * v10);
+        o.val[0] = x_bits(v11);
+        o.ent = NO_ROW;
+        return true;
+    }
+};
+extern "C" __global__ __launch_bounds__(256) void xk_group_tight(XArgs a, XGroup<P::NV>::Args s, int64_t nrows, int64_t seg_rows, int nseg) {
+    x_queue8<P, XGroup, false>(a, s, nrows, seg_rows, nseg);
+}
```

New measurement: 451.9 billion rows/s (median of 6 runs). Within noise of the previous version (+1.2%).
